# yuecideng/Misc3D

Measured on AMD Instinct MI355X. Metric: RANSAC hypotheses/sec, 1M-pt cloud (inlier-score GB/s: roofline.algorithmic_reuse), higher is better.
Workload: dtype f64 decisions (fp32 screen + fp64 recount)

## Files before the change

### include/misc3d_amd.h

```cpp
#ifndef MISC3D_AMD_H
#define MISC3D_AMD_H

#include <stddef.h>
#include <stdint.h>

#ifdef __cplusplus
extern "C" {
#endif

#define M3D_OK 1
#define M3D_FALSE 0
#define M3D_ERR_PROBABILITY (-1)
#define M3D_ERR_TOO_FEW_POINTS (-2)
#define M3D_ERR_NO_NORMALS (-3)
#define M3D_ERR_SIZE_MISMATCH (-4)
#define M3D_ERR_INVALID_ARG (-5)
#define M3D_ERR_DEVICE (-6)
#define M3D_ERR_INTERNAL (-7)
#define M3D_ERR_NON_FINITE (-8)

enum m3d_model_kind { M3D_PLANE = 0, M3D_SPHERE = 1, M3D_CYLINDER = 2 };

typedef struct m3d_stats {
    double fitness;
// ... 354 lines not shown
    uint64_t n_nodes;
    uint64_t n_rays;
    uint64_t pair_tests;
    uint64_t nodes_visited;
} m3d_raycast_stats;
int m3d_raycast_pinhole(const m3d_raycast_mesh *meshes, size_t n_meshes, const double *poses, size_t n_poses, size_t n_frames,
                        int width, int height, double fx, double fy, double cx, double cy, int device, float *t_hit,
                        uint32_t *geometry_ids, uint32_t *primitive_ids, float *primitive_normals, m3d_raycast_stats *stats);

int m3d_match_mutual_nn(const double *feat_src, size_t n_src, const double *feat_dst, size_t n_dst,
                        int dim, int method, int n_trees, int device, size_t *out_src,
                        size_t *out_dst, size_t *k);
uint64_t m3d_match_last_fallbacks(void);

typedef struct m3d_comm m3d_comm;
#define M3D_COMM_ID_BYTES 128
int m3d_comm_unique_id(uint8_t id[M3D_COMM_ID_BYTES]);
m3d_comm *m3d_comm_create_rccl(const uint8_t id[M3D_COMM_ID_BYTES], int world, int rank, int device);
typedef int (*m3d_allgather_fn)(void *user, const void *send, void *recv, size_t bytes_per_rank);
m3d_comm *m3d_comm_create_host(int world, int rank, m3d_allgather_fn fn, void *user);
int m3d_comm_create_local(int world, m3d_comm **comms );
void m3d_comm_destroy(m3d_comm *comm);
int m3d_comm_world(const m3d_comm *comm);
int m3d_comm_rank(const m3d_comm *comm);
uint64_t m3d_comm_collectives(const m3d_comm *comm);

int m3d_cloud_fit_sharded(m3d_cloud *cloud, m3d_comm *comm, int kind, double threshold, size_t max_iteration,
                          double probability, const uint64_t *seed, double *params, size_t *inliers,
                          size_t *n_inliers, m3d_stats *stats);
int m3d_segment_plane_iterative_sharded(const double *xyz, size_t n, double threshold, int max_iteration,
                                        double min_ratio, const uint64_t *seed, int device, m3d_comm *comm,
                                        size_t max_clusters, double *planes, size_t *cluster_offsets,
                                        size_t *cluster_indices, size_t *n_clusters);
int m3d_segment_plane_iterative_multi(const double *xyz, size_t n, double threshold, int max_iteration,
                                      double min_ratio, const uint64_t *seed, const int *devices, int n_dev,
                                      size_t max_clusters, double *planes, size_t *cluster_offsets,
                                      size_t *cluster_indices, size_t *n_clusters);
int m3d_fit_multi(int kind, const double *xyz, const double *normals, size_t n, double threshold,
                  size_t max_iteration, double probability, const uint64_t *seed, const int *devices, int n_dev,
                  double *params, size_t *inliers, size_t *n_inliers, m3d_stats *stats);
int m3d_registration_ransac_sharded(const double *src, size_t n_src, const double *dst, size_t n_dst,
                                    const size_t *corr_src, const size_t *corr_dst, size_t m, double threshold,
                                    int max_iter, double edge_length_threshold, double confidence,
                                    const uint64_t *seed, int device, m3d_comm *comm, double T[16],
                                    m3d_reg_stats *stats);

typedef struct m3d_config {
    int32_t dense_scoring;
    int32_t speculative_refine;
    int32_t lead_hypotheses;
    int32_t score_groups_per_block;
    int32_t score_min_workgroups;
    int32_t dense_workgroups;
    int32_t reg_neighbour_lists;
    int32_t reg_prune;
    int32_t match_brute;
    int32_t match_fp32_screen;
    int32_t pool_limit_mb;
    int32_t kernel_timing;
    int32_t reg_sorted_lists;
    int32_t score_fp32_screen;
    int32_t cull_fp32;
    int32_t reg_fp32_screen;
    int32_t sorted_tombstones;
    int32_t score_mfma;
    int32_t score_mfma_groups;
    int32_t score_waves4;
    int32_t score_waves4_groups;
    int32_t score_phases;
    int32_t compact_one_pass;
    int32_t plane_bound;
    int32_t lanes;
    int32_t wait_spin_us;
    int32_t prestream;
    int32_t chunk_cap;
    int32_t first_chunk;
    int32_t reg_cells_per_radius;
    int32_t match_pipeline;
    int32_t reg_cache;
    int32_t device_aliases;
    int32_t lanes_eager;
    int32_t list_mask;
    int32_t mask_early;
} m3d_config;
void m3d_get_config(m3d_config *out);
int m3d_set_config(const m3d_config *in);

const char *m3d_last_error(void);
int m3d_device_count(void);
const char *m3d_version(void);

#ifdef __cplusplus
}
#endif
#endif
```

### include/misc3d_amd_bench.h

```cpp
#ifndef MISC3D_AMD_BENCH_H
#define MISC3D_AMD_BENCH_H

#include "misc3d_amd.h"

#ifdef __cplusplus
extern "C" {
#endif

int m3d_bench_time_score(m3d_cloud *cloud, int kind, double threshold, const uint32_t *samples,
                         size_t n_hypotheses, int reps, int mode, double *ms_avg,
                         uint64_t *listed_pairs);


int m3d_bench_fp64_issue_rate(int device, double ms_target, double *tera_lane_ops_per_s, double *ms_measured);

int m3d_bench_cloud_setup_ms(const m3d_cloud *cloud, double out[5]);

int m3d_bench_plane_upper_bounds(m3d_cloud *cloud, double threshold, const uint32_t *samples, size_t n_hypotheses,
                                 uint32_t *ub_out);
int m3d_bench_upper_bounds(m3d_cloud *cloud, int kind, double threshold, const uint32_t *samples, size_t n_hypotheses,
                           uint32_t *ub_out);
int m3d_bench_last_segment_ms(double out[6]);

int m3d_bench_reg_checkers(const double *ps, const double *pd, const double *T, double edge_threshold,
                           double distance_threshold);

int m3d_bench_kabsch_sums(const double *src, const double *dst, size_t n, int device, double out[18]);

int m3d_bench_icp_sums(const double *src, size_t n_src, const double *dst, size_t n_dst, double max_correspondence_distance,
                       const double *T, int device, double out[29], int64_t *corr);

int m3d_bench_fps_force_path(int path);

int m3d_bench_knn_force_path(int path);

int m3d_bench_voxel_force_path(int path);

int m3d_bench_proximity_cutoffs(double dist, double angle_deg, double out[5]);

int m3d_bench_fpfh_pair_bins(const double *pairs, size_t m, int32_t *bins, double *features);

unsigned m3d_bench_match_last_path(void);

#ifdef __cplusplus
}
#endif
#endif
```

### misc3d_amd/capi.py

```python
from __future__ import annotations

import ctypes as C
import threading
import os
import sys
from dataclasses import dataclass

import numpy as np

_HERE = os.path.dirname(os.path.abspath(__file__))
FP_ORDER = int(os.environ.get("M3D_FP_ORDER", "0") or 0)
_VARIANT = os.environ.get("M3D_LIB_VARIANT", "")
LIB_PATH = os.path.join(_HERE, "lib", *([_VARIANT] if _VARIANT else ([f"order{FP_ORDER}"] if FP_ORDER else [])), "libmisc3d_amd.so")
HEADER_PATH = os.path.join(os.path.dirname(_HERE), "include", "misc3d_amd.h")

PLANE, SPHERE, CYLINDER = 0, 1, 2
MINIMAL_SAMPLE = {PLANE: 3, SPHERE: 4, CYLINDER: 2}
NUM_PARAMS = {PLANE: 4, SPHERE: 4, CYLINDER: 7}
MODEL_STRIDE = 8

OK, FALSE = 1, 0
ERR_PROBABILITY, ERR_TOO_FEW_POINTS, ERR_NO_NORMALS, ERR_SIZE_MISMATCH = -1, -2, -3, -4
ERR_INVALID_ARG, ERR_DEVICE, ERR_INTERNAL = -5, -6, -7
ERR_NON_FINITE = -8
# ... 149 lines not shown
                                                  C.c_void_p, C.c_void_p]
        L.m3d_bench_voxel_force_path.argtypes = [C.c_int]
        L.m3d_raycast_pinhole.argtypes = [C.c_void_p, C.c_size_t, C.c_void_p, C.c_size_t, C.c_size_t, C.c_int, C.c_int, C.c_double,
                                          C.c_double, C.c_double, C.c_double, C.c_int, C.c_void_p, C.c_void_p, C.c_void_p,
                                          C.c_void_p, C.c_void_p]
        L.m3d_proximity_segment.argtypes = [C.c_void_p, C.c_void_p, C.c_size_t, C.c_size_t, C.c_double, C.c_void_p,
                                            C.c_size_t, C.c_size_t, C.c_int, C.c_void_p, C.c_void_p, C.c_void_p, C.c_void_p,
                                            C.c_void_p]
        L.m3d_proximity_segment_nn.argtypes = [C.c_void_p, C.c_void_p, C.c_size_t, C.c_size_t, C.c_size_t, C.c_void_p,
                                               C.c_void_p, C.c_void_p, C.c_size_t, C.c_size_t, C.c_int, C.c_void_p,
                                               C.c_void_p, C.c_void_p, C.c_void_p, C.c_void_p]
        L.m3d_radius_neighbors.argtypes = [C.c_void_p, C.c_size_t, C.c_double, C.c_int, C.c_void_p, C.c_void_p, C.c_void_p,
                                           C.c_size_t, C.c_void_p]
        L.m3d_bench_proximity_cutoffs.argtypes = [C.c_double, C.c_double, C.c_void_p]
        L.m3d_knn_create.restype = C.c_void_p
        L.m3d_knn_create.argtypes = [C.c_void_p, C.c_size_t, C.c_int, C.c_int, C.c_void_p]
        L.m3d_knn_destroy.restype = None
        L.m3d_knn_destroy.argtypes = [C.c_void_p]
        L.m3d_knn_size.restype = C.c_size_t
        L.m3d_knn_size.argtypes = [C.c_void_p]
        L.m3d_knn_dim.argtypes = [C.c_void_p]
        L.m3d_knn_search.argtypes = [C.c_void_p, C.c_void_p, C.c_size_t, C.c_int, C.c_int64, C.c_double, C.c_size_t,
                                     C.c_void_p, C.c_void_p, C.c_void_p, C.c_void_p, C.c_void_p]
        L.m3d_bench_knn_force_path.argtypes = [C.c_int]
        L.m3d_estimate_normals.argtypes = [C.c_void_p, C.c_size_t, C.c_int, C.c_double, C.c_int, C.c_int, C.c_void_p, C.c_int,
                                           C.c_void_p, C.c_void_p]
        L.m3d_compute_fpfh.argtypes = [C.c_void_p, C.c_void_p, C.c_size_t, C.c_int, C.c_double, C.c_int, C.c_int, C.c_void_p,
                                       C.c_void_p]
        L.m3d_preprocess_fragment.argtypes = [C.c_void_p, C.c_void_p, C.c_size_t, C.c_double, C.c_int, C.c_void_p, C.c_void_p,
                                              C.c_void_p]
        L.m3d_bench_fpfh_pair_bins.argtypes = [C.c_void_p, C.c_size_t, C.c_void_p, C.c_void_p]
        L.m3d_match_last_fallbacks.restype = C.c_uint64
        L.m3d_match_last_fallbacks.argtypes = []
        L.m3d_match_mutual_nn.argtypes = [C.c_void_p, C.c_size_t, C.c_void_p, C.c_size_t, C.c_int, C.c_int, C.c_int,
                                          C.c_int, C.c_void_p, C.c_void_p, C.c_void_p]
        L.m3d_comm_unique_id.argtypes = [C.c_void_p]
        L.m3d_comm_create_rccl.restype = C.c_void_p
        L.m3d_comm_create_rccl.argtypes = [C.c_void_p, C.c_int, C.c_int, C.c_int]
        L.m3d_comm_create_host.restype = C.c_void_p
        L.m3d_comm_create_host.argtypes = [C.c_int, C.c_int, ALLGATHER_FN, C.c_void_p]
        L.m3d_comm_create_local.argtypes = [C.c_int, C.c_void_p]
        L.m3d_comm_destroy.restype = None
        L.m3d_comm_destroy.argtypes = [C.c_void_p]
        L.m3d_comm_world.argtypes = [C.c_void_p]
        L.m3d_comm_rank.argtypes = [C.c_void_p]
        L.m3d_comm_collectives.restype = C.c_uint64
        L.m3d_comm_collectives.argtypes = [C.c_void_p]
        L.m3d_cloud_fit_sharded.argtypes = [C.c_void_p, C.c_void_p, C.c_int, C.c_double, C.c_size_t, C.c_double, C.c_void_p,
                                            C.c_void_p, C.c_void_p, C.c_void_p, C.c_void_p]
        L.m3d_segment_plane_iterative_clouds.argtypes = [C.c_void_p, C.c_size_t, C.c_double, C.c_int, C.c_double,
                                                          C.c_void_p, C.c_int, C.c_size_t, C.c_void_p, C.c_void_p,
                                                          C.c_void_p, C.c_void_p, C.c_void_p]
        L.m3d_segment_plane_iterative_sharded.argtypes = [C.c_void_p, C.c_size_t, C.c_double, C.c_int, C.c_double,
                                                          C.c_void_p, C.c_int, C.c_void_p, C.c_size_t, C.c_void_p,
                                                          C.c_void_p, C.c_void_p, C.c_void_p]
        L.m3d_segment_plane_iterative_multi.argtypes = [C.c_void_p, C.c_size_t, C.c_double, C.c_int, C.c_double,
                                                        C.c_void_p, C.c_void_p, C.c_int, C.c_size_t, C.c_void_p,
                                                        C.c_void_p, C.c_void_p, C.c_void_p]
        L.m3d_fit_multi.argtypes = [C.c_int, C.c_void_p, C.c_void_p, C.c_size_t, C.c_double, C.c_size_t, C.c_double,
                                    C.c_void_p, C.c_void_p, C.c_int, C.c_void_p, C.c_void_p, C.c_void_p, C.c_void_p]
        L.m3d_registration_ransac_sharded.argtypes = [C.c_void_p, C.c_size_t, C.c_void_p, C.c_size_t, C.c_void_p,
                                                      C.c_void_p, C.c_size_t, C.c_double, C.c_int, C.c_double,
                                                      C.c_double, C.c_void_p, C.c_int, C.c_void_p, C.c_void_p,
                                                      C.c_void_p]
        L.m3d_bench_fp64_issue_rate.argtypes = [C.c_int, C.c_double, C.c_void_p, C.c_void_p]
        L.m3d_bench_cloud_setup_ms.argtypes = [C.c_void_p, C.c_void_p]
        L.m3d_bench_last_segment_ms.argtypes = [C.c_void_p]
        L.m3d_bench_reg_checkers.argtypes = [C.c_void_p, C.c_void_p, C.c_void_p, C.c_double, C.c_double]
        L.m3d_get_config.restype = None
        L.m3d_get_config.argtypes = [C.c_void_p]
        L.m3d_set_config.argtypes = [C.c_void_p]
        L.m3d_release_cached.restype = None
        L.m3d_release_cached.argtypes = [C.c_int]
        _lib = L
    return _lib


class Config(C.Structure):
    _fields_ = [(k, C.c_int32) for k in ("dense_scoring", "speculative_refine", "lead_hypotheses",
                                         "score_groups_per_block", "score_min_workgroups", "dense_workgroups",
                                         "reg_neighbour_lists", "reg_prune", "match_brute", "match_fp32_screen",
                                         "pool_limit_mb", "kernel_timing", "reg_sorted_lists", "score_fp32_screen",
                                         "cull_fp32", "reg_fp32_screen", "sorted_tombstones", "score_mfma", "score_mfma_groups", "score_waves4", "score_waves4_groups", "score_phases", "compact_one_pass", "plane_bound",
                                         "lanes", "wait_spin_us", "prestream", "chunk_cap", "first_chunk", "reg_cells_per_radius", "match_pipeline", "reg_cache", "device_aliases", "lanes_eager", "list_mask", "mask_early")]


def fp64_issue_rate(device=0, ms_target=2.0):
    t, ms = C.c_double(0), C.c_double(0)
    _check(lib().m3d_bench_fp64_issue_rate(device, ms_target, C.cast(C.byref(t), C.c_void_p), C.cast(C.byref(ms), C.c_void_p)))
    return float(t.value), float(ms.value)


def match_last_path() -> int:
    f = lib().m3d_bench_match_last_path
    f.restype = C.c_uint
    f.argtypes = []
    return int(f())


def get_config() -> Config:
    c = Config()
    lib().m3d_get_config(C.byref(c))
    return c


def set_config(**kw) -> Config:
    old = get_config()
    new = get_config()
    for k, v in kw.items():
        if not hasattr(new, k):
            raise AttributeError(k)
        setattr(new, k, int(v))
    _check(lib().m3d_set_config(C.byref(new)))
    return old


def restore_config(cfg: Config):
    _check(lib().m3d_set_config(C.byref(cfg)))


class Comm:

    def __init__(self, handle, keep=None):
        if not handle:
            raise M3DError(ERR_DEVICE, last_error())
        self._h = handle
        self._keep = keep

    @classmethod
    def rccl(cls, group=None, device=0, world=None, rank=None):
        import torch
        import torch.distributed as dist
        if world is None:
            world, rank = (dist.get_world_size(group), dist.get_rank(group)) if dist.is_initialized() else (1, 0)
        ident = np.zeros(128, dtype=np.uint8)
        status = np.zeros(129, dtype=np.uint8)
        err = None
        if rank == 0:
            try:
                _check(lib().m3d_comm_unique_id(_p(ident)))
                status[:128] = ident
                status[128] = 1
            except M3DError as e:
                err = e
        if world > 1:
            t = torch.from_numpy(status)
            dist.broadcast(t, src=dist.get_global_rank(group, 0) if group is not None else 0, group=group)
        if not status[128]:
            raise err if err is not None else M3DError(-6, "rank 0 could not create an RCCL unique id")
        ident = np.ascontiguousarray(status[:128])
        libc = C.CDLL(None)
        sys.stdout.flush()
        libc.fflush(None)
        if os.environ.get("M3D_RCCL_KEEP_STDOUT") == "1":
            return cls(lib().m3d_comm_create_rccl(_p(ident), world, rank, device))
        saved = os.dup(1)
        os.dup2(2, 1)
        try:
            h = lib().m3d_comm_create_rccl(_p(ident), world, rank, device)
        finally:
            libc.fflush(None)
            os.dup2(saved, 1)
            os.close(saved)
        return cls(h)

    @classmethod
    def host(cls, world, rank, fn):
# ... 219 lines not shown
            try:
                self._inl_buf = np.asarray(_PinnedU64(n))
            except MemoryError:
                self._inl_buf = np.empty(n, dtype=np.uint64)
        return self._inl_buf

    def close(self):
        if getattr(self, "_h", None):
            lib().m3d_cloud_destroy(self._h)
            self._h = None
        self._inl_buf = None

    def __del__(self):
        try:
            self.close()
        except Exception:
            pass

    def __enter__(self):
        return self

    def __exit__(self, *a):
        self.close()

    def fit(self, kind, threshold=0.01, max_iteration=1000, probability=0.9999, seed=None,
            want_inliers=True, copy=True) -> Fit:
        params = np.zeros(NUM_PARAMS[kind])
        inl = None
        if want_inliers:
            inl = _seg_scratch(max(self.n_created, 1)) if copy else None
            if inl is None:
                inl = self._out_buf()
        ni = C.c_size_t(0)
        st = Stats()
        _s, sref = _seed_ref(seed)
        rc = _check(lib().m3d_cloud_fit(self._h, kind, threshold, max_iteration, probability, sref, _addr(params),
                                        _addr(inl), C.byref(ni), C.byref(st)))
        if want_inliers:
            inliers = inl[: ni.value].copy() if copy else inl[: ni.value]
        else:
            inliers = np.zeros(0, dtype=np.uint64)
        return Fit(rc, params, inliers, (st, ni.value))

    def fit_sharded(self, comm, kind, threshold=0.01, max_iteration=1000, probability=0.9999, seed=None,
                    want_inliers=True, copy=True) -> Fit:
        params = np.zeros(NUM_PARAMS[kind])
        inl = self._out_buf() if want_inliers else None
        ni = C.c_size_t(0)
        st = Stats()
        _s, sref = _seed_ref(seed)
        rc = _check(lib().m3d_cloud_fit_sharded(self._h, comm._h if comm is not None else None, kind, threshold,
                                                max_iteration, probability, sref, _addr(params), _addr(inl),
                                                C.byref(ni), C.byref(st)))
        if want_inliers:
            inliers = inl[: ni.value].copy() if copy else inl[: ni.value]
        else:
            inliers = np.zeros(0, dtype=np.uint64)
        return Fit(rc, params, inliers, (st, ni.value))

    def score_range(self, kind, threshold, samples, begin=0, end=None, want_models=True):
        samples = np.ascontiguousarray(samples, dtype=np.uint32).reshape(-1, MINIMAL_SAMPLE[kind])
        end = len(samples) if end is None else end
        cnt = np.empty(end - begin, dtype=np.uint32)
        val = np.empty(end - begin, dtype=np.uint8)
        mod = np.empty((end - begin, MODEL_STRIDE)) if want_models else None
        _check(lib().m3d_cloud_score_range(self._h, kind, threshold, _p(samples), begin, end, _p(cnt), _p(val),
                                           _p(mod)))
        return val, (mod[:, : NUM_PARAMS[kind]].copy() if want_models else None), cnt

    def time_score(self, kind, threshold, samples, reps=5, mode=0):
        samples = np.ascontiguousarray(samples, dtype=np.uint32).reshape(-1, MINIMAL_SAMPLE[kind])
        ms = C.c_double(0)
        listed = C.c_uint64(0)
        _check(lib().m3d_bench_time_score(self._h, kind, threshold, _p(samples), len(samples), reps, mode,
                                          C.cast(C.byref(ms), C.c_void_p), C.cast(C.byref(listed), C.c_void_p)))
        return float(ms.value), int(listed.value)

    def plane_upper_bounds(self, threshold, samples):
        samples = np.ascontiguousarray(samples, dtype=np.uint32).reshape(-1, 3)
        ub = np.zeros(len(samples), dtype=np.uint32)
        _check(lib().m3d_bench_plane_upper_bounds(self._h, threshold, _p(samples), len(samples), _p(ub)))
        return ub

    def upper_bounds(self, kind, threshold, samples):
        samples = np.ascontiguousarray(samples, dtype=np.uint32).reshape(-1, MINIMAL_SAMPLE[kind])
        ub = np.zeros(len(samples), dtype=np.uint32)
        _check(lib().m3d_bench_upper_bounds(self._h, kind, threshold, _p(samples), len(samples), _p(ub)))
        return ub

    def exact_error(self, kind, threshold, model):
        model = _f64(model)
        cnt = C.c_uint64(0)
        err = C.c_double(0)
        _check(lib().m3d_cloud_exact_error(self._h, kind, threshold, _p(model), C.cast(C.byref(cnt), C.c_void_p),
                                           C.cast(C.byref(err), C.c_void_p)))
        return int(cnt.value), float(err.value)

    refine_takes_expected = True

    def refine(self, kind, threshold, params, copy=True, expected=None):
        params = _f64(params).copy()
        inl = self._out_buf()
        ni = C.c_size_t(0)
        rc = _check(lib().m3d_cloud_refine_expect(self._h, kind, threshold, _p(params),
                                                  -1 if expected is None else int(expected), _p(inl),
                                                  C.cast(C.byref(ni), C.c_void_p)))
        return rc, params, (inl[: ni.value].copy() if copy else inl[: ni.value])

    def minimal_model(self, kind, threshold, sample_row):
        row = np.ascontiguousarray(sample_row, dtype=np.uint32).reshape(-1)
        if self.n == self.n_created:
            pts = np.ascontiguousarray(self._host_xyz[row])
            nrm = np.ascontiguousarray(self._host_nrm[row]) if self._host_nrm is not None else None
            model = np.zeros(8)
            ok = C.c_uint8(0)
            _check(lib().m3d_minimal_fit(kind, _p(pts), _p(nrm), _p(model), C.cast(C.byref(ok), C.c_void_p)))
            return model[: NUM_PARAMS[kind]].copy()
        _, mod, _ = self.score_range(kind, threshold, row.reshape(1, -1), 0, 1)
        return mod[0]

    def remove_inliers(self, kind, threshold, model):
        model = _f64(model).copy()
        nr = C.c_size_t(0)
        _check(lib().m3d_cloud_remove_inliers(self._h, kind, threshold, _p(model), C.cast(C.byref(nr), C.c_void_p)))
        self.n = int(lib().m3d_cloud_size(self._h))
        return nr.value


def draw_samples(n_points, kind, n_hyp, seed):
    out = np.zeros((n_hyp, MINIMAL_SAMPLE[kind]), dtype=np.uint32)
    _check(lib().m3d_draw_samples(n_points, kind, n_hyp, C.c_uint64(seed), _p(out)))
    return out


def fit(kind, xyz, normals=None, threshold=0.01, max_iteration=1000, probability=0.9999, seed=None,
        device=0, copy=True) -> Fit:
    xyz = _f64(xyz).reshape(-1, 3)
    n = len(xyz)
    params = np.zeros(NUM_PARAMS[kind])
    inl = _seg_scratch(max(n, 1))
    if inl is None:
        inl = np.empty(max(n, 1), dtype=np.uint64)
    ni = C.c_size_t(0)
    st = Stats()
    _s, sref = _seed_ref(seed)
    sp = C.cast(sref, C.c_void_p) if sref else None
    nip, stp = C.cast(C.byref(ni), C.c_void_p), C.cast(C.byref(st), C.c_void_p)
    if kind == CYLINDER:
        nrm = _f64(normals).reshape(-1, 3) if normals is not None else None
        rc = lib().m3d_fit_cylinder(_p(xyz), _p(nrm), n, threshold, max_iteration, probability, sp, device,
                                    _p(params), _p(inl), nip, stp)
    else:
        fn = lib().m3d_fit_plane if kind == PLANE else lib().m3d_fit_sphere
        rc = fn(_p(xyz), n, threshold, max_iteration, probability, sp, device, _p(params), _p(inl), nip, stp)
    _check(rc)
    d = st.asdict()
    d["n_inliers"] = int(ni.value)
    return Fit(rc, params, inl[: ni.value].copy() if copy else inl[: ni.value], d)


_seg_tls = threading.local()
_SEG_SCRATCH_MAX = 1 << 25


def _seg_scratch(n):
    if n > _SEG_SCRATCH_MAX:
# ... 931 lines not shown
```

### misc3d_amd/csrc/m3d_bound.hip

```cpp
#include "m3d_cull_kernels.hpp"

#include <cstdlib>

#include "m3d_bound_fp.hpp"
#include "m3d_config.hpp"
#include "m3d_eig3.hpp"
#include "m3d_fp.hpp"
#include "m3d_wave.hpp"

#pragma clang fp contract(off)

namespace m3d {

constexpr int kFrameLevels = 12;

__global__ __launch_bounds__(64) void tile_frames_k(const double* __restrict__ sx, const double* __restrict__ sy,
                                                     const double* __restrict__ sz, uint32_t n_tiles,
                                                     double* __restrict__ frames, uint16_t* __restrict__ cum) {
    __shared__ float pf[3][kTilePoints];
    __shared__ uint32_t hist[kBoundBins + 2];
    const int lane = threadIdx.x;
    const uint32_t tile = blockIdx.x;
    if (tile >= n_tiles) return;
    constexpr int P = kTilePoints / 64;
// ... 98 lines not shown
        for (int j = 0; j < P; ++j) {
            const double dx = px[j] - c[0], dy = py[j] - c[1], dz = pz[j] - c[2];
            const double w = (dx * e[0] + dy * e[1]) + dz * e[2];
            if (fin[j] && fabs(w) < band) {
                m[0] += 1.0;
                m[1] += dx; m[2] += dy; m[3] += dz;
                m[4] += dx * dx; m[5] += dx * dy; m[6] += dx * dz;
                m[7] += dy * dy; m[8] += dy * dz; m[9] += dz * dz;
            }
        }
#pragma unroll
        for (int k = 0; k < 10; ++k) m[k] = wave_sum(m[k]);
        if (!(m[0] >= 8.0)) break;
        const double in = 1.0 / m[0];
        const double mx = m[1] * in, my = m[2] * in, mz = m[3] * in;
        const double A[9] = {m[4] * in - mx * mx, m[5] * in - mx * my, m[6] * in - mx * mz,
                             m[5] * in - mx * my, m[7] * in - my * my, m[8] * in - my * mz,
                             m[6] * in - mx * mz, m[8] * in - my * mz, m[9] * in - mz * mz};
        double en[3];
        j3x3_smallest_eigvec(A, en);
        if (!((en[0] + en[1] + en[2]) * 0.0 == 0.0)) break;
        e[0] = en[0]; e[1] = en[1]; e[2] = en[2];
        c[0] += mx; c[1] += my; c[2] += mz;
        const double q = (e[0] * (A[0] * e[0] + A[1] * e[1] + A[2] * e[2]) + e[1] * (A[3] * e[0] + A[4] * e[1] + A[5] * e[2])) +
                         e[2] * (A[6] * e[0] + A[7] * e[1] + A[8] * e[2]);
        s = sqrt(fmax(q, 0.0));
        s = fmax(s, 1e-7 * ext);
        band = 3.5 * s;
    }
    const int kmin = (fabs(e[0]) <= fabs(e[1]) && fabs(e[0]) <= fabs(e[2])) ? 0 : (fabs(e[1]) <= fabs(e[2]) ? 1 : 2);
    const double a3[3] = {kmin == 0 ? 1.0 : 0.0, kmin == 1 ? 1.0 : 0.0, kmin == 2 ? 1.0 : 0.0};
    double u[3] = {e[1] * a3[2] - e[2] * a3[1], e[2] * a3[0] - e[0] * a3[2], e[0] * a3[1] - e[1] * a3[0]};
    const double ul = sqrt((u[0] * u[0] + u[1] * u[1]) + u[2] * u[2]);
    u[0] /= ul; u[1] /= ul; u[2] /= ul;
    const double v[3] = {e[1] * u[2] - e[2] * u[1], e[2] * u[0] - e[0] * u[2], e[0] * u[1] - e[1] * u[0]};
    const double wlo = -5.0 * s, invd = (double)kBoundBins / (10.0 * s);
    double U = 0.0, V = 0.0, W = 0.0, R = 0.0;
#pragma unroll
    for (int j = 0; j < P; ++j) {
        if (!fin[j]) continue;
        const double dx = px[j] - c[0], dy = py[j] - c[1], dz = pz[j] - c[2];
        const double w = (dx * e[0] + dy * e[1]) + dz * e[2];
        const double uu = (dx * u[0] + dy * u[1]) + dz * u[2];
        const double vv = (dx * v[0] + dy * v[1]) + dz * v[2];
        const double rx = ((dx - w * e[0]) - uu * u[0]) - vv * v[0];
        const double ry = ((dy - w * e[1]) - uu * u[1]) - vv * v[1];
        const double rz = ((dz - w * e[2]) - uu * u[2]) - vv * v[2];
        U = fmax(U, fabs(uu));
        V = fmax(V, fabs(vv));
        W = fmax(W, fabs(w));
        R = fmax(R, fmax(fabs(rx), fmax(fabs(ry), fabs(rz))));
        atomicAdd(&hist[bound_bin(w, wlo, invd)], 1u);
    }
    U = wave_max(U);
    V = wave_max(V);
    W = wave_max(W);
    R = wave_max(R);
    __syncthreads();
    {
        const uint32_t h0 = hist[2 * lane], h1 = hist[2 * lane + 1];
        const uint32_t own = h0 + h1, incl = wave_incl_scan(own, lane);
        const uint32_t excl = incl - own;
        cm[2 * lane] = (uint16_t)excl;
        cm[2 * lane + 1] = (uint16_t)(excl + h0);
        if (lane == 63) cm[kBoundBins + 2] = (uint16_t)incl;
    }
    const double Rm = R + 1e-13 * (mabs + ext);
    const bool ok = (U + V + W + Rm) < 1e12 && invd > 0.0 && invd < 1e30 && ext > 1e-12 && mabs < 1e12;
    if (lane == 0) {
        fr[0] = c[0]; fr[1] = c[1]; fr[2] = c[2];
        fr[3] = e[0]; fr[4] = e[1]; fr[5] = e[2];
        fr[6] = u[0]; fr[7] = u[1]; fr[8] = u[2];
        fr[9] = v[0]; fr[10] = v[1]; fr[11] = v[2];
        fr[12] = U; fr[13] = V; fr[14] = Rm; fr[15] = wlo; fr[16] = invd; fr[17] = W; fr[18] = nf;
        fr[19] = ok ? 1.0 : 0.0;
    }
}

void launch_tile_frames(const SortedView& s, double* frames, uint16_t* cum, hipStream_t st) {
    if (s.n_tiles) tile_frames_k<<<s.n_tiles, 64, 0, st>>>(s.x, s.y, s.z, s.n_tiles, frames, cum);
}

constexpr int kBoundWaves = 8;
template <int KIND , int kBoundTpw >
__global__ __launch_bounds__(64 * kBoundWaves) void plane_bound_k(const double* __restrict__ frames, const uint16_t* __restrict__ cum,
                                                                   uint32_t n_tiles, double max_abs,
                                                                   const double* __restrict__ score,
                                                                   const unsigned long long* __restrict__ masks, uint32_t n_groups,
                                                                   const double* __restrict__ boxes, const float* __restrict__ cull32,
                                                                   uint32_t* __restrict__ surv_count,
                                                                   const uint32_t* __restrict__ surv,
                                                                   uint32_t* __restrict__ ubsum, const uint32_t* __restrict__ best_count,
                                                                   unsigned long long* __restrict__ keep,
                                                                   uint32_t* __restrict__ tickets ,
                                                                   uint32_t max_list) {
    constexpr int kBoundTpb = kBoundWaves * kBoundTpw;
    __shared__ float bx_s[kBoundTpb][6];
    __shared__ double c_s[kBoundTpb][3];
    __shared__ float f_s[kBoundTpb][kFrameStride];
    __shared__ __attribute__((aligned(8))) uint16_t cm_s[kBoundTpb][kCumStride];
    __shared__ uint32_t wsum[kBoundWaves][64];
    __shared__ double rec_s[64][9];
    __shared__ float q_s[64][13];
    const int lane = threadIdx.x & 63;
    const int wave = __builtin_amdgcn_readfirstlane((int)(threadIdx.x >> 6));
    const uint32_t total = surv_count[0];
    if (total > max_list) {
        if (blockIdx.x == 0 && blockIdx.y == 0 && threadIdx.x == 0) surv_count[0] = 0u;
        return;
    }
    if (blockIdx.x * 64u >= total) return;
    const uint32_t t0 = blockIdx.y * (uint32_t)kBoundTpb, nt = min((uint32_t)kBoundTpb, n_tiles - t0);
    {
        const double* __restrict__ src = frames + (size_t)t0 * kFrameStride;
        for (uint32_t i = threadIdx.x; i < nt * (uint32_t)kFrameStride; i += 64u * kBoundWaves) {
            const uint32_t tl = i / (uint32_t)kFrameStride, k = i % (uint32_t)kFrameStride;
            const double v = src[i];
            if (k < 3u) c_s[tl][k] = v;
            f_s[tl][k] = frame_to_f32(v, k);
        }
        if (KIND != 0) {
            __syncthreads();
            if (threadIdx.x < nt) f_s[threadIdx.x][0] = cyl_tile_rho(f_s[threadIdx.x]);
        }
        if (cull32)
            for (uint32_t i = threadIdx.x; i < nt * 6u; i += 64u * kBoundWaves)
                bx_s[i / 6u][i % 6u] = reinterpret_cast<const float*>(boxes + (size_t)(t0 + i / 6u) * kBoxStride + 8)[i % 6u];
        const uint32_t* __restrict__ csrc = reinterpret_cast<const uint32_t*>(cum + (size_t)t0 * kCumStride);
        uint32_t* cdst = reinterpret_cast<uint32_t*>(&cm_s[0][0]);
        for (uint32_t i = threadIdx.x; i < nt * (uint32_t)(kCumStride / 2); i += 64u * kBoundWaves) cdst[i] = csrc[i];
    }
    for (uint32_t first = blockIdx.x * 64u; first < total; first += gridDim.x * 64u) {
        const uint32_t nb = min(64u, total - first);
        const bool has = (uint32_t)lane < nb;
        const uint32_t h = surv[first + (has ? (uint32_t)lane : 0u)];
        __syncthreads();
        {
            const uint32_t k = threadIdx.x & 7u;
#pragma unroll
            for (uint32_t si = threadIdx.x >> 3; si < 64u; si += (64u * kBoundWaves) >> 3) {
                const uint32_t hh = surv[first + min(si, nb - 1u)];
                rec_s[si][k] = score[(size_t)hh * kModelStride + k];
                if (cull32) {
                    q_s[si][k] = cull32[(size_t)(hh >> 1) * 24u + (hh & 1u) + 2u * k];
                    if (KIND == 2 && k < 3u) q_s[si][8u + k] = cull32[(size_t)(hh >> 1) * 24u + (hh & 1u) + 2u * (8u + k)];
                }
            }
        }
        __syncthreads();
        PlaneBoundRec pr;
        CylBoundRec cr;
        if (KIND == 0) {
            pr = plane_bound_record(rec_s[lane], max_abs);
            pr.ok = pr.ok && has;
        } else {
            cr = KIND == 1 ? sphere_bound_record(rec_s[lane], max_abs) : cyl_bound_record(rec_s[lane], max_abs);
            cr.ok = cr.ok && has;
        }
        const unsigned long long bit = 1ull << (h & 63u);
        const unsigned long long* __restrict__ mrow = masks + (size_t)(h >> 6);
        bool tch[kBoundTpw];
        float q[11] = {0, 0, 0, 0, 0, 0, 0, 0, 0, 0, 0};
        if (cull32) {
#pragma unroll
            for (int k = 0; k < (KIND == 2 ? 11 : 8); ++k) q[k] = q_s[lane][k];
        } else {
#pragma unroll
            for (int i = 0; i < kBoundTpw; ++i) {
                const uint32_t tl = (uint32_t)(wave + kBoundWaves * i);
                tch[i] = (has && tl < nt) ? (mrow[(size_t)(t0 + tl) * n_groups] & bit) != 0ull : false;
            }
        }
        uint32_t ub = 0;
#pragma unroll
        for (int i = 0; i < kBoundTpw; ++i) {
            const int tl = wave + kBoundWaves * i;
            if (cull32 && KIND == 0) {
                const float* bx = bx_s[tl];
                const float sv = __builtin_fmaf(q[0], bx[0], __builtin_fmaf(q[1], bx[1], __builtin_fmaf(q[2], bx[2], q[3])));
                const float hx = __builtin_fmaxf(bx[3], 0.0f), hy = __builtin_fmaxf(bx[4], 0.0f), hz = __builtin_fmaxf(bx[5], 0.0f);
                const float rv = __builtin_fmaf(q[4], hx, __builtin_fmaf(q[5], hy, __builtin_fmaf(q[6], hz, q[7])));
                tch[i] = has && (uint32_t)tl < nt && bx[3] >= 0.0f && !(rv - __builtin_fabsf(sv) < 0.0f);
            } else if (cull32 && KIND == 2) {
                const float* bx = bx_s[tl];
                const bool live = bx[3] >= 0.0f;
                const float hx = live ? bx[3] : 0.0f, hy = live ? bx[4] : 0.0f, hz = live ? bx[5] : 0.0f;
                const float rb = __builtin_sqrtf(__builtin_fmaf(hz, hz, __builtin_fmaf(hy, hy, hx * hx))) * 1.000001f;
                const float d1 = __builtin_fmaf(q[0], bx[0], __builtin_fmaf(q[1], bx[1], __builtin_fmaf(q[2], bx[2], q[3])));
                const float d2 = __builtin_fmaf(q[4], bx[0], __builtin_fmaf(q[5], bx[1], __builtin_fmaf(q[6], bx[2], q[7])));
                const float tt = __builtin_fmaf(d2, d2, d1 * d1);
                const float dist = __builtin_sqrtf(tt);
                const float rt = q[8] * rb;
                const float t1 = (q[9] + rt) - dist;
                const float t2 = (dist + rt) - q[10];
                const float t = __uint_as_float(__float_as_uint(t1) | __float_as_uint(t2));
                tch[i] = has && (uint32_t)tl < nt && live && !(t < 0.0f);
            }
            if (__ballot(tch[i]) == 0ull) continue;
            const uint32_t u_t = KIND == 0 ? plane_pair_ub(pr, c_s[tl], f_s[tl], cm_s[tl])
                                           : cyl_pair_ub(cr, c_s[tl], f_s[tl], f_s[tl][0], cm_s[tl]);
            ub += tch[i] ? u_t : 0u;
        }
        wsum[wave][lane] = ub;
        __syncthreads();
        if (wave == 0) {
            uint32_t tot = 0;
#pragma unroll
            for (int w = 0; w < kBoundWaves; ++w) tot += wsum[w][lane];
            if (has && tot) atomicAdd(&ubsum[h], tot);
            __threadfence();
            const uint32_t blk = first / 64u;
            uint32_t old = 0;
            if (lane == 0) old = atomicAdd(&tickets[1u + blk], 1u);
            old = (uint32_t)__builtin_amdgcn_readfirstlane((int)old);
            if (old == gridDim.y - 1u) {
                __threadfence();
                const uint32_t best = best_count[0];
                const uint32_t sum = has ? atomicAdd(&ubsum[h], 0u) : 0u;
                if (has && best != 0u && sum < best) atomicAnd(&keep[h >> 6], ~bit);
                uint32_t done = 0;
                if (lane == 0) {
                    tickets[1u + blk] = 0u;
                    done = atomicAdd(&tickets[0], 1u);
                    if (done == (total + 63u) / 64u - 1u) {
                        tickets[0] = 0u;
                        surv_count[0] = 0u;
                    }
                }
            }
        }
    }
}

constexpr int kCylTpb = 64;
__global__ __launch_bounds__(64 * kBoundWaves) void cyl_bound_words_k(const double* __restrict__ frames, const uint16_t* __restrict__ cum,
                                                                       uint32_t n_tiles, double max_abs, const double* __restrict__ score,
                                                                       uint32_t* __restrict__ surv_count, const uint32_t* __restrict__ surv,
                                                                       uint32_t* __restrict__ ubsum, const uint32_t* __restrict__ best_count,
                                                                       unsigned long long* __restrict__ keep, uint32_t* __restrict__ tickets,
                                                                       uint32_t max_list, const unsigned long long* __restrict__ touched,
                                                                       uint32_t touched_stride) {
    __shared__ double c_s[kCylTpb][3];
    __shared__ float f_s[kCylTpb][kFrameStride];
    __shared__ __attribute__((aligned(8))) uint16_t cm_s[kCylTpb][kCumStride];
    const int lane = threadIdx.x & 63;
    const uint32_t wave = threadIdx.x >> 6;
    const uint32_t total = surv_count[0];
    if (total > max_list) {
        if (blockIdx.x == 0 && blockIdx.y == 0 && threadIdx.x == 0) surv_count[0] = 0u;
        return;
    }
    if (blockIdx.x * (64u * kBoundWaves) >= total) return;
    const uint32_t t0 = blockIdx.y * (uint32_t)kCylTpb, nt = min((uint32_t)kCylTpb, n_tiles - t0);
    {
        const double* __restrict__ src = frames + (size_t)t0 * kFrameStride;
        for (uint32_t i = threadIdx.x; i < nt * (uint32_t)kFrameStride; i += 64u * kBoundWaves) {
            const uint32_t tl = i / (uint32_t)kFrameStride, k = i % (uint32_t)kFrameStride;
            const double v = src[i];
            if (k < 3u) c_s[tl][k] = v;
            f_s[tl][k] = frame_to_f32(v, k);
        }
        __syncthreads();
        if (threadIdx.x < nt) f_s[threadIdx.x][0] = cyl_tile_rho(f_s[threadIdx.x]);
        const uint32_t* __restrict__ csrc = reinterpret_cast<const uint32_t*>(cum + (size_t)t0 * kCumStride);
        uint32_t* cdst = reinterpret_cast<uint32_t*>(&cm_s[0][0]);
        for (uint32_t i = threadIdx.x; i < nt * (uint32_t)(kCumStride / 2); i += 64u * kBoundWaves) cdst[i] = csrc[i];
        __syncthreads();
    }
    for (uint32_t first = (blockIdx.x * kBoundWaves + wave) * 64u; first < total; first += gridDim.x * (64u * kBoundWaves)) {
        const uint32_t nb = min(64u, total - first);
        const bool has = (uint32_t)lane < nb;
        const uint32_t h = surv[first + (has ? (uint32_t)lane : 0u)];
        double rec[8];
        {
            const double2* __restrict__ rp = reinterpret_cast<const double2*>(score + (size_t)h * kModelStride);
#pragma unroll
            for (int k = 0; k < 4; ++k) {
                const double2 v = rp[k];
                rec[2 * k] = v.x;
                rec[2 * k + 1] = v.y;
            }
        }
        CylBoundRec cr = cyl_bound_record(rec, max_abs);
        cr.ok = cr.ok && has;
        unsigned long long w0 = has ? touched[(size_t)(t0 / 64u) * touched_stride + h] : 0ull;
        unsigned long long w1 = (has && t0 + 64u < n_tiles) ? touched[(size_t)(t0 / 64u + 1u) * touched_stride + h] : 0ull;
        uint32_t ub = 0;
        for (uint32_t tl = 0; tl < nt; ++tl) {
            const bool mine = (((tl < 64u ? w0 : w1) >> (tl & 63u)) & 1ull) != 0ull;
            if (__builtin_amdgcn_ballot_w64(mine) == 0ull) continue;
            const uint32_t u_t = cyl_pair_ub(cr, c_s[tl], f_s[tl], f_s[tl][0], cm_s[tl]);
            ub += mine ? u_t : 0u;
        }
        if (has && ub) atomicAdd(&ubsum[h], ub);
        __threadfence();
        const uint32_t blk = first / 64u;
        uint32_t old = 0;
        if (lane == 0) old = atomicAdd(&tickets[1u + blk], 1u);
        old = (uint32_t)__builtin_amdgcn_readfirstlane((int)old);
        if (old == gridDim.y - 1u) {
            __threadfence();
            const uint32_t best = best_count[0];
            const uint32_t sum = has ? atomicAdd(&ubsum[h], 0u) : 0u;
            if (has && best != 0u && sum < best) atomicAnd(&keep[h >> 6], ~(1ull << (h & 63u)));
            if (lane == 0) {
                tickets[1u + blk] = 0u;
                const uint32_t done = atomicAdd(&tickets[0], 1u);
                if (done == (total + 63u) / 64u - 1u) {
                    tickets[0] = 0u;
                    surv_count[0] = 0u;
                }
            }
        }
    }
}

void launch_plane_bound(int kind, const SortedView& s, const double* score, const unsigned long long* masks, unsigned long long* keep,
                        uint32_t n_groups, uint32_t group_begin, uint32_t group_end, uint32_t* ubsum,
                        const uint32_t* best_count, uint32_t* surv_count, const uint32_t* surv, uint32_t* tickets,
                        const float* cull32, hipStream_t st, bool always, const unsigned long long* touched, uint32_t touched_stride) {
    group_end = std::min(group_end, n_groups);
    if (!s.frames || !s.frame_cum || !s.n_tiles || !surv || !surv_count || !tickets || group_begin >= group_end) return;
    const uint32_t window = group_end - group_begin;
    constexpr uint32_t gdiv = 6;
    const uint32_t gx = std::min<uint32_t>(window, std::max<uint32_t>(4u, (window + gdiv - 1) / gdiv));
    constexpr int tpw = 8, tpw_cyl = 16;
    const uint32_t tpb = (uint32_t)(kBoundWaves * (kind == 0 ? tpw : tpw_cyl));
    const uint32_t max_list = always ? 0xFFFFFFFFu : window * 32u;
    if (kind == 2 && touched && s.radius < 1e18) {
        const dim3 gw((window + kBoundWaves - 1) / kBoundWaves, (s.n_tiles + kCylTpb - 1) / kCylTpb);
        cyl_bound_words_k<<<gw, 64 * kBoundWaves, 0, st>>>(s.frames, s.frame_cum, s.n_tiles, s.max_abs, score, surv_count, surv, ubsum, best_count,
                                                           keep, tickets, max_list, touched, touched_stride);
        return;
    }
    const dim3 g(gx, (s.n_tiles + tpb - 1) / tpb), b(64 * kBoundWaves);
    if (s.radius >= 1e18 || kind == 1) cull32 = nullptr;
    auto go = [&](auto kernel) {
        kernel<<<g, b, 0, st>>>(s.frames, s.frame_cum, s.n_tiles, s.max_abs, score, masks, n_groups, s.boxes, cull32, surv_count, surv,
                                ubsum, best_count, keep, tickets, max_list);
    };
    if (kind == 0) go(plane_bound_k<0, tpw>);
    else if (kind == 1) go(plane_bound_k<1, tpw_cyl>);
    else go(plane_bound_k<2, tpw_cyl>);
}

}
```

### misc3d_amd/csrc/m3d_bound_fp.hpp

```cpp
#pragma once
#include <math.h>
#include <stdint.h>

#if defined(__HIPCC__)
#include <hip/hip_runtime.h>
#ifndef M3D_HD
#define M3D_HD __host__ __device__ __forceinline__
#endif
#else
#ifndef M3D_HD
#define M3D_HD inline
#endif
#endif

namespace m3d {

constexpr int kFrameStride = 20;
constexpr int kBoundBins = 126;
constexpr int kCumStride = 132;
constexpr int kBoundTilePoints = 512;

M3D_HD int bound_bin(double w, double wlo, double invd) {
    const double t = floor((w - wlo) * invd);
    return (int)fmin(fmax(t, -1.0), (double)kBoundBins) + 1;
// ... 95 lines not shown
    return r;
}
M3D_HD CylBoundRec sphere_bound_record(const double* rec , double max_abs) {
    CylBoundRec r;
    const double Wm = 2.0 * max_abs + ((fabs(rec[0]) + fabs(rec[1])) + fabs(rec[2]));
    const double Es = 1e-12 * (Wm * Wm);
    const double slo = rec[3], shi = rec[4];
    r.ok = (slo == slo) && (shi == shi) && (shi >= 0.0) && (Wm < 1e12) && (shi < 1e30);
    for (int k = 0; k < 3; ++k) {
        r.p1[k] = rec[k];
        r.df[k] = 0.0f;
    }
    const double dhi = sqrt(shi + Es) * (1.0 + 1e-12);
    const double sl = slo - Es;
    const double dlo = sl > 0.0 ? sqrt(sl) * (1.0 - 1e-12) : 0.0;
    r.dhif = (float)(dhi * (1.0 + 1e-6));
    r.dlof = (float)(dlo * (1.0 - 1e-6));
    r.mg = (float)(1e-13 * Wm * (1.0 + 1e-6));
    return r;
}
M3D_HD float bound_sqrt(float x) {
#if defined(__HIP_DEVICE_COMPILE__)
    return __builtin_amdgcn_sqrtf(x);
#else
    return sqrtf(x);
#endif
}
M3D_HD float cyl_tile_rho(const float* f) {
    const float U = f[12], V = f[13], R = f[14], W = f[17];
    return __builtin_fmaf(bound_sqrt(__builtin_fmaf(W, W, __builtin_fmaf(U, U, V * V))), 1.0001f, 1.75f * R);
}
template <class CumPtr>
M3D_HD uint32_t cyl_pair_ub(const CylBoundRec& r, const double* c3, const float* f, float rho, CumPtr cm) {
    const float U = f[12], V = f[13], R = f[14], W = f[17];
    const bool framed = f[19] != 0.0f && r.ok;
    const float v0 = (float)(c3[0] - r.p1[0]), v1 = (float)(c3[1] - r.p1[1]), v2 = (float)(c3[2] - r.p1[2]);
    const float v1n = (__builtin_fabsf(v0) + __builtin_fabsf(v1)) + __builtin_fabsf(v2);
    const float k = __builtin_fmaf(v0, r.df[0], __builtin_fmaf(v1, r.df[1], v2 * r.df[2]));
    const float m0 = __builtin_fmaf(-k, r.df[0], v0), m1 = __builtin_fmaf(-k, r.df[1], v1), m2 = __builtin_fmaf(-k, r.df[2], v2);
    const float f2 = __builtin_fmaf(m0, m0, __builtin_fmaf(m1, m1, m2 * m2));
    const float fc = bound_sqrt(f2);
    const float eabs = 2e-6f * v1n;
    const bool one_side = fc - eabs > rho * 1.001f && f2 < 1e30f && f2 > 1e-30f;
    const float inv = bound_rcp(fc);
    const float nx = m0 * inv, ny = m1 * inv, nz = m2 * inv;
    const float n1 = 1.7321f, e32 = 5e-7f * 1.7321f;
    const float g0 = __builtin_fmaf(nx, f[3], __builtin_fmaf(ny, f[4], nz * f[5]));
    const float nu = __builtin_fmaf(nx, f[6], __builtin_fmaf(ny, f[7], nz * f[8]));
    const float nv = __builtin_fmaf(nx, f[9], __builtin_fmaf(ny, f[10], nz * f[11]));
    const float hif = r.dhif - fc;
    const float rho1 = rho * 1.0001f;
    const float q2 = __builtin_fmaf(r.dlof, r.dlof, -(rho1 * rho1)) - 3e-7f * (r.dlof * r.dlof);
    const bool has_lo = q2 > 1e-30f;
    const float lof = has_lo ? bound_sqrt(q2) * (1.0f - 3e-7f) - fc : 0.0f;
    float aa = __builtin_fmaf(__builtin_fabsf(nu) + e32, U,
                              __builtin_fmaf(__builtin_fabsf(nv) + e32, V, __builtin_fmaf(n1, R, __builtin_fmaf(e32, W, r.mg + eabs))));
    aa = __builtin_fmaf(aa, 1.00001f, 1e-5f * ((__builtin_fabsf(hif) + __builtin_fabsf(lof)) + aa));
#ifdef M3D_BOUND_NO_SLACK
    aa = 0.0f;
#endif
    const float ninf = -__builtin_huge_valf();
    const float g = __builtin_fabsf(g0);
    const float a_lo = g0 < 0.0f ? -hif : (has_lo ? lof : ninf), a_hi = g0 < 0.0f ? (has_lo ? -lof : -ninf) : hif;
    const float ig = bound_rcp(g);
    float Lw = (a_lo - aa) * ig, Hw = (a_hi + aa) * ig;
    Lw -= 1e-5f * __builtin_fabsf(Lw);
    Hw += 1e-5f * __builtin_fabsf(Hw);
    const float wlo = f[15], invd = f[16];
#ifdef M3D_BOUND_NO_SLACK
    const float out = 0.0f;
#else
    const float out = 1.0f;
#endif
    const float tL = __builtin_floorf((Lw - wlo) * invd) - out, tH = __builtin_floorf((Hw - wlo) * invd) + out;
    const bool whole = !(tL == tL) || !(tH == tH) || !one_side;
    const int bl = (int)__builtin_fminf(__builtin_fmaxf(whole ? 0.0f : tL, -1.0f), (float)kBoundBins) + 1;
    const int bh = (int)__builtin_fminf(__builtin_fmaxf(whole ? 0.0f : tH, -1.0f), (float)kBoundBins) + 1;
    const int lo_c = (int)cm[bl], hi_c = (int)cm[bh + 1];
    uint32_t u_t = (uint32_t)(hi_c > lo_c ? hi_c - lo_c : 0);
    u_t = whole ? (uint32_t)f[18] : u_t;
    return framed ? u_t : (uint32_t)kBoundTilePoints;
}

}
```

### misc3d_amd/csrc/m3d_config.cpp

```cpp
#include "m3d_config.hpp"

#include <algorithm>
#include <cstdlib>
#include <cstring>
#include <mutex>

#include "m3d_driver.hpp"

namespace m3d {
namespace {
m3d_config g_cfg;
std::once_flag g_once;
std::mutex g_cfg_mu;
thread_local m3d_config t_cfg;
thread_local int t_cfg_pins = 0;

long env_long(const char* name, long def) {
    const char* e = std::getenv(name);
    if (!e || !*e) return def;
    char* end = nullptr;
    const long v = std::strtol(e, &end, 10);
    return end == e ? def : v;
}
bool env_is(const char* name, char first) {
    const char* e = std::getenv(name);
    return e && e[0] == first;
}
void sanitize(m3d_config& c) {
    if (c.lead_hypotheses < 64 || c.lead_hypotheses % 64) c.lead_hypotheses = 128;
    if (c.score_groups_per_block < 1 || c.score_groups_per_block > 64) c.score_groups_per_block = 8;
    if (c.score_min_workgroups < 1) c.score_min_workgroups = 8192;
    if (c.dense_workgroups < 1) c.dense_workgroups = 8192;
    if (c.pool_limit_mb < 0) c.pool_limit_mb = 0;
    if (c.score_phases < -1 || c.score_phases == 1 || c.score_phases > 3) c.score_phases = -1;
    if (c.plane_bound < 0 || c.plane_bound > 2) c.plane_bound = 1;
    if (c.cull_fp32 < 0 || c.cull_fp32 > 2) c.cull_fp32 = 1;
    c.score_mfma = c.score_mfma_groups = c.score_waves4 = c.score_waves4_groups = c.compact_one_pass = 0;
    if (c.lanes < 1 || c.lanes > 8) c.lanes = 4;
    if (c.wait_spin_us < 0) c.wait_spin_us = 500;
    c.prestream = c.prestream != 0;
    c.chunk_cap = (int32_t)std::min<long>(std::max<long>(((long)c.chunk_cap + 63) / 64 * 64, 1024), 262144);
    c.first_chunk = c.first_chunk <= 0 ? 0 : (int32_t)std::min<long>(((long)c.first_chunk + 63) / 64 * 64, 1 << 20);
    if (c.reg_cells_per_radius < 1 || c.reg_cells_per_radius > 16) c.reg_cells_per_radius = 4;
    if (c.match_pipeline < 0 || c.match_pipeline > 2) c.match_pipeline = 1;
    if (c.reg_cache < 0 || c.reg_cache > 2) c.reg_cache = 1;
    if (c.device_aliases < 0) c.device_aliases = 0;
    if (c.device_aliases > 16) c.device_aliases = 16;
    if (c.lanes_eager < 1 || c.lanes_eager > 8) c.lanes_eager = 2;
    if (c.list_mask < 0) c.list_mask = 1;
    if (c.list_mask > 16) c.list_mask = 16;
    c.mask_early = c.mask_early != 0;
}
void load_env() {
    std::memset(&g_cfg, 0, sizeof(g_cfg));
    g_cfg.dense_scoring = env_is("M3D_DENSE", '1');
    g_cfg.speculative_refine = !env_is("M3D_SPEC", '0');
    g_cfg.lead_hypotheses = (int32_t)env_long("M3D_LEAD", 128);
    g_cfg.score_groups_per_block = (int32_t)env_long("M3D_GPB", 8);
    g_cfg.score_min_workgroups = (int32_t)env_long("M3D_SCORE_MIN_WGS", 8192);
    g_cfg.dense_workgroups = (int32_t)env_long("M3D_SCORE_WGS", 8192);
    g_cfg.reg_neighbour_lists = !env_is("M3D_REG_NL", '0');
    g_cfg.reg_prune = !env_is("M3D_REG_PRUNE", '0');
    g_cfg.match_brute = env_is("M3D_MATCH_BRUTE", '1');
    g_cfg.match_fp32_screen = env_is("M3D_MATCH_SCREEN", 'f');
    g_cfg.pool_limit_mb = (int32_t)env_long("M3D_POOL_MB", 4096);
    g_cfg.kernel_timing = env_is("M3D_KERNEL_TIMING", '1');
    g_cfg.reg_sorted_lists = !env_is("M3D_REG_SORTED", '0');
    g_cfg.score_fp32_screen = !env_is("M3D_SCORE_SCREEN", '0');
    g_cfg.cull_fp32 = env_is("M3D_CULL_FP32", '0') ? 0 : (env_is("M3D_CULL_FP32", '2') ? 2 : 1);
    g_cfg.reg_fp32_screen = !env_is("M3D_REG_SCREEN", '0');
    g_cfg.sorted_tombstones = !env_is("M3D_TOMBSTONES", '0');
    g_cfg.score_phases = (int32_t)env_long("M3D_SCORE_PHASES", -1);
    g_cfg.plane_bound = (int32_t)env_long("M3D_PLANE_BOUND", 1);
    g_cfg.lanes = (int32_t)env_long("M3D_LANES", 4);
    g_cfg.wait_spin_us = (int32_t)env_long("M3D_SPIN_US", 500);
    g_cfg.prestream = !env_is("M3D_PRESTREAM", '0');
    g_cfg.chunk_cap = (int32_t)env_long("M3D_CHUNK_CAP", 24576);
    g_cfg.first_chunk = (int32_t)env_long("M3D_FIRST_CHUNK", 2048);
    g_cfg.reg_cells_per_radius = (int32_t)env_long("M3D_REG_K", 4);
    g_cfg.match_pipeline = (int32_t)env_long("M3D_MATCH_PIPELINE", 1);
    g_cfg.reg_cache = (int32_t)env_long("M3D_REG_CACHE", 1);
    g_cfg.device_aliases = (int32_t)env_long("M3D_DEVICE_ALIASES", 0);
    g_cfg.lanes_eager = (int32_t)env_long("M3D_LANES_EAGER", 2);
    g_cfg.list_mask = (int32_t)env_long("M3D_LIST_MASK", 1);
    g_cfg.mask_early = !env_is("M3D_MASK_EARLY", '0');
    sanitize(g_cfg);
}
}

const m3d_config& config() {
    std::call_once(g_once, load_env);
    if (t_cfg_pins > 0) return t_cfg;
    std::lock_guard<std::mutex> lock(g_cfg_mu);
    t_cfg = g_cfg;
    return t_cfg;
}
void config_pin() {
    std::call_once(g_once, load_env);
    if (t_cfg_pins++ == 0) {
        std::lock_guard<std::mutex> lock(g_cfg_mu);
        t_cfg = g_cfg;
    }
}
void config_unpin() {
    if (t_cfg_pins > 0) --t_cfg_pins;
}
void config_store(const m3d_config& c) {
    std::call_once(g_once, load_env);
    m3d_config n = c;
    sanitize(n);
    std::lock_guard<std::mutex> lock(g_cfg_mu);
    g_cfg = n;
}
}

extern "C" {
void m3d_get_config(m3d_config* out) {
    if (out) *out = m3d::config();
}
int m3d_set_config(const m3d_config* in) {
    if (!in) return m3d::fail(M3D_ERR_INVALID_ARG, "invalid argument");
    if (in->score_mfma || in->score_waves4 || in->compact_one_pass)
        return m3d::fail(M3D_ERR_INVALID_ARG, "score_mfma / score_waves4 / compact_one_pass: retired, must be 0 (the variants were removed)");
    m3d::config_store(*in);
    return M3D_OK;
}
}
```

### misc3d_amd/csrc/m3d_cull_kernels.hip

```cpp
#include "m3d_cull_kernels.hpp"
#include "m3d_poison.hpp"

#include <hip/hip_ext.h>

#include <cstdlib>
#include <type_traits>

#include "m3d_config.hpp"
#include "m3d_fp.hpp"
#include "m3d_tile_count.hpp"
#include "m3d_wave.hpp"

#pragma clang fp contract(off)

namespace m3d {

typedef float f32x2 __attribute__((ext_vector_type(2)));

__global__ __launch_bounds__(256) void tile_boxes_k(const double* __restrict__ sx, const double* __restrict__ sy,
                                                     const double* __restrict__ sz, uint32_t n_tiles,
                                                     double* __restrict__ boxes, double ox, double oy, double oz,
                                                     float* __restrict__ tile_f32) {
    const int lane = threadIdx.x & 63;
    const uint32_t tile = blockIdx.x * 4u + (threadIdx.x >> 6);
    if (tile >= n_tiles) return;
    double lo[3] = {INFINITY, INFINITY, INFINITY}, hi[3] = {-INFINITY, -INFINITY, -INFINITY};
    double pts[kTilePoints / 64][3];
#pragma unroll
    for (int j = 0; j < kTilePoints / 64; ++j) {
        const size_t i = (size_t)tile * kTilePoints + j * 64 + lane;
        const double p[3] = {sx[i], sy[i], sz[i]};
        for (int k = 0; k < 3; ++k) {
            pts[j][k] = p[k];
            lo[k] = fmin(lo[k], p[k]);
            hi[k] = fmax(hi[k], p[k]);
        }
    }
    for (int off = 32; off > 0; off >>= 1)
        for (int k = 0; k < 3; ++k) {
            lo[k] = fmin(lo[k], __shfl_xor(lo[k], off, 64));
            hi[k] = fmax(hi[k], __shfl_xor(hi[k], off, 64));
        }
    bool finite = true;
    if (tile_f32) {
        const bool empty_t = !(lo[0] <= hi[0]);
        f32x2* __restrict__ t2 = reinterpret_cast<f32x2*>(tile_f32 + (size_t)tile * kTileF32Floats);
#pragma unroll
        for (int k = 0; k < 3; ++k) {
            const double c = empty_t ? 0.0 : 0.5 * lo[k] + 0.5 * hi[k];
#pragma unroll
            for (int j = 0; j < kTilePoints / 128; ++j) {
                const f32x2 v = {(float)(pts[2 * j][k] - c), (float)(pts[2 * j + 1][k] - c)};
                t2[(k * (kTilePoints / 128) + j) * 64 + lane] = v;
                finite = finite && (v.x * 0.0f == 0.0f) && (v.y * 0.0f == 0.0f);
            }
        }
    }
    const bool screenable = tile_f32 && __ballot(!finite) == 0ull;
    if (lane == 0) {
        double* b = boxes + (size_t)tile * kBoxStride;
        const bool empty = !(lo[0] <= hi[0]);
        for (int k = 0; k < 3; ++k) {
            const double c = 0.5 * lo[k] + 0.5 * hi[k];
            b[k] = empty ? 0.0 : c;
            b[3 + k] = empty ? -1.0 : fmax(hi[k] - c, c - lo[k]) * (1.0 + 1e-12) + 1e-300;
        }
        b[6] = screenable ? 1.0 : 0.0;
        b[7] = 0.0;
        float* f = reinterpret_cast<float*>(b + 8);
        const double o[3] = {ox, oy, oz};
        for (int k = 0; k < 3; ++k) {
            const double cr = b[k] - o[k];
            const float c32 = (float)cr;
            const double hh = (b[3 + k] + fabs(cr - (double)c32)) * (1.0 + 1e-6) + 1e-30;
            f[k] = empty ? 0.0f : c32;
            f[3 + k] = empty ? -1.0f : f32_round_up(hh);
        }
        const float hx = empty ? 0.0f : f[3], hy = empty ? 0.0f : f[4], hz = empty ? 0.0f : f[5];
        f[6] = __builtin_sqrtf(__builtin_fmaf(hz, hz, __builtin_fmaf(hy, hy, hx * hx))) * 1.000001f;
        f[7] = 0.0f;
    }
}

void launch_tile_boxes(const SortedView& s, double* boxes, hipStream_t st) {
    if (s.n_tiles) tile_boxes_k<<<(s.n_tiles + 3) / 4, 256, 0, st>>>(s.x, s.y, s.z, s.n_tiles, boxes, s.origin[0], s.origin[1], s.origin[2], s.tile_f32);
}

__global__ __launch_bounds__(256) void poison_plane_inliers_k(PoisonJob job) {
    poison_tile(job, blockIdx.x * 4u + (threadIdx.x >> 6), (int)(threadIdx.x & 63));
}
PoisonJob make_poison_job(const SortedView& s, const double* model, double thr, uint32_t* total) {
    PoisonJob j;
// ... 338 lines not shown
    if (!s.n_tiles || group_begin >= group_end) return;
    const uint32_t window = group_end - group_begin;
    if (ub && !ub_is_zero) (void)hipMemsetAsync(ub + (size_t)group_begin * 64, 0, sizeof(uint32_t) * (size_t)window * 64, st);
    const uint32_t tblocks = (s.n_tiles + 63) / 64;
    uint32_t gpw = std::max<uint32_t>(1, (uint32_t)(((uint64_t)tblocks * window) / 8192));
    gpw = std::min<uint32_t>(gpw, 8);
    const dim3 g(tblocks, (window + gpw - 1) / gpw), b(64);
    if (cull32 && s.radius < 1e18 && config().cull_fp32 != 0) {
        if (window >= 128u && config().cull_fp32 != 2) {
            const uint32_t tpw = 64u;
            const dim3 gh((s.n_tiles + tpw - 1) / tpw, window);
            if (kind == 0) cull_hyp32_k<0><<<gh, b, 0, st>>>(s.boxes, s.n_tiles, cull32, n_groups, tpw, masks, ub, group_begin, group_end, ubp, touched, touched_stride);
            else if (kind == 1) cull_hyp32_k<1><<<gh, b, 0, st>>>(s.boxes, s.n_tiles, cull32, n_groups, tpw, masks, ub, group_begin, group_end, ubp, touched, touched_stride);
            else cull_hyp32_k<2><<<gh, b, 0, st>>>(s.boxes, s.n_tiles, cull32, n_groups, tpw, masks, ub, group_begin, group_end, ubp, touched, touched_stride);
            if (touched_written) *touched_written = touched != nullptr;
            return;
        }
        if (kind == 0)
            cull_tiles32_k<0><<<g, b, 0, st>>>(s.boxes, s.n_tiles, cull32, n_groups, gpw, masks, ub, group_begin, group_end, ubp);
        else if (kind == 1)
            cull_tiles32_k<1><<<g, b, 0, st>>>(s.boxes, s.n_tiles, cull32, n_groups, gpw, masks, ub, group_begin, group_end, ubp);
        else
            cull_tiles32_k<2><<<g, b, 0, st>>>(s.boxes, s.n_tiles, cull32, n_groups, gpw, masks, ub, group_begin, group_end, ubp);
        return;
    }
    if (kind == 0)
        cull_tiles_k<0><<<g, b, 0, st>>>(s.boxes, s.n_tiles, score, n_groups, gpw, masks, ub, group_begin, group_end);
    else if (kind == 1)
        cull_tiles_k<1><<<g, b, 0, st>>>(s.boxes, s.n_tiles, score, n_groups, gpw, masks, ub, group_begin, group_end);
    else
        cull_tiles_k<2><<<g, b, 0, st>>>(s.boxes, s.n_tiles, score, n_groups, gpw, masks, ub, group_begin, group_end);
}

struct SurvOut {
    uint32_t* count = nullptr;
    uint32_t* ids = nullptr;
};
__device__ __forceinline__ void emit_survivors(const SurvOut surv, unsigned long long m, bool k, uint32_t h) {
    if (!surv.count || !m) return;
    uint32_t base = 0;
    if (threadIdx.x == 0) base = atomicAdd(surv.count, (uint32_t)__popcll(m));
    base = (uint32_t)__builtin_amdgcn_readfirstlane((int)base);
    const uint32_t rank = __builtin_amdgcn_mbcnt_hi((uint32_t)(m >> 32), __builtin_amdgcn_mbcnt_lo((uint32_t)m, 0u));
    if (k) surv.ids[base + rank] = h;
}
__global__ __launch_bounds__(64) void keep_mask_k(const uint32_t* __restrict__ ub,
                                                   const uint32_t* __restrict__ best_count_ptr,
                                                   unsigned long long* __restrict__ keep,
                                                   uint32_t* __restrict__ zero, uint32_t rep_stride,
                                                   uint32_t group_offset, SurvOut surv) {
    const uint32_t g = group_offset + blockIdx.x;
    const uint32_t h = g * 64u + threadIdx.x;
    const uint32_t best = best_count_ptr ? best_count_ptr[0] : 0u;
    const bool k = !ub || best == 0 || (uint64_t)ub[h] * kTilePoints >= best;
    const unsigned long long m = __ballot(k);
    if (threadIdx.x == 0) keep[g] = m;
    emit_survivors(surv, m, k, h);
    if (zero) {
#pragma unroll
        for (int r = 0; r < kCountReplicas; ++r) zero[(size_t)r * rep_stride + h] = 0u;
        if (blockIdx.x == 0)
            for (int i = threadIdx.x; i < kPairReplicas; i += 64) zero[(size_t)kCountReplicas * rep_stride + i] = 0u;
    }
}
void launch_keep_mask(const uint32_t* ub, const uint32_t* best_count, uint32_t n_groups, unsigned long long* keep,
                      hipStream_t st, uint32_t* zero_counts_rep, uint32_t rep_stride, uint32_t group_offset, uint32_t* surv_count, uint32_t* surv) {
    if (!n_groups) return;
    if (!ub && !zero_counts_rep && !surv_count) {
        (void)hipMemsetAsync(keep + group_offset, 0xFF, sizeof(unsigned long long) * n_groups, st);
        return;
    }
    keep_mask_k<<<n_groups, 64, 0, st>>>(ub, best_count, keep, zero_counts_rep, rep_stride, group_offset, SurvOut{surv_count, surv});
}

__global__ __launch_bounds__(64) void lead_fold_keep_k(const uint32_t* __restrict__ counts_rep, uint32_t rep_stride,
                                                        uint32_t lead, const uint8_t* __restrict__ valid, uint32_t h_count,
                                                        uint32_t* __restrict__ records, uint32_t* __restrict__ best_count,
                                                        const uint32_t* __restrict__ ub,
                                                        unsigned long long* __restrict__ keep,
                                                        uint32_t* __restrict__ zero, uint32_t group_offset,
                                                        uint32_t* __restrict__ records_dev,
                                                        unsigned long long* __restrict__ pick_key,
                                                        unsigned long long* __restrict__ pick_key2,
                                                        SurvOut surv) {
    const uint32_t g = group_offset + blockIdx.x;
    const uint32_t prev = best_count[0];
    uint32_t v = 0;
    unsigned long long key = 0, key2 = 0;
    for (uint32_t h = threadIdx.x; h < lead; h += 64u) {
        uint32_t c = 0;
#pragma unroll
        for (int r = 0; r < kCountReplicas; ++r) c += counts_rep[(size_t)r * rep_stride + h];
        const bool ok = h < h_count && valid[h];
        if (blockIdx.x == 0) {
            if (records) records[h] = c | (ok ? 0x80000000u : 0u);
            if (records_dev) records_dev[h] = c | (ok ? 0x80000000u : 0u);
        }
        v = max(v, ok ? c : 0u);
        if (ok && c) key = max(key, ((unsigned long long)c << 32) | (0xFFFFFFFFu - h));
        if (ok && c) key2 = max(key2, ((unsigned long long)c << 32) | h);
    }
    v = wave_max(v);
    if (blockIdx.x == 0 && threadIdx.x == 0 && v) atomicMax(best_count, v);
    if (zero && blockIdx.x == 0) {
        uint32_t* __restrict__ pair_rep = zero + (size_t)kCountReplicas * rep_stride;
        uint32_t p = 0;
        for (int r = threadIdx.x; r < kPairMain; r += 64) p += pair_rep[r];
        p = wave_sum(p);
        if (threadIdx.x == 0) pair_rep[kPairLead] = p;
    }
    if (pick_key && blockIdx.x == 0) {
        key = wave_max(key);
        if (threadIdx.x == 0 && key) atomicMax(pick_key, key);
        if (pick_key2) {
            key2 = wave_max(key2);
            if (threadIdx.x == 0 && key2) atomicMax(pick_key2, key2);
        }
    }
    const uint32_t best = max(prev, v);
    const uint32_t h = g * 64u + threadIdx.x;
    const bool k = !ub || best == 0 || (uint64_t)ub[h] * kTilePoints >= best;
    const unsigned long long m = __ballot(k);
    if (threadIdx.x == 0) keep[g] = m;
    emit_survivors(surv, m, k, h);
    if (zero) {
#pragma unroll
        for (int r = 0; r < kCountReplicas; ++r) zero[(size_t)r * rep_stride + h] = 0u;
    }
}
void launch_lead_fold_keep(const uint32_t* counts_rep, uint32_t rep_stride, uint32_t lead, const uint8_t* valid,
                           uint32_t h_count, uint32_t* records, uint32_t* best_count, const uint32_t* ub,
                           unsigned long long* keep, uint32_t n_groups_rest, hipStream_t st, uint32_t* records_dev,
                           uint32_t group_begin, unsigned long long* pick_key, unsigned long long* pick_key2, uint32_t* surv_count, uint32_t* surv) {
    if (group_begin == 0xFFFFFFFFu) group_begin = lead / 64u;
    if (!n_groups_rest) return;
    lead_fold_keep_k<<<n_groups_rest, 64, 0, st>>>(counts_rep, rep_stride, lead, valid, h_count, records, best_count, ub,
                                                   keep, const_cast<uint32_t*>(counts_rep), group_begin, records_dev, pick_key, pick_key2, SurvOut{surv_count, surv});
}

template <int KIND>
__global__ __launch_bounds__(64) void score_mask_k(const double* __restrict__ sx, const double* __restrict__ sy,
                                                    const double* __restrict__ sz,
                                                    const double* __restrict__ score,
                                                    const unsigned long long* __restrict__ masks,
                                                    const unsigned long long* __restrict__ keep,
                                                    uint32_t n_groups ,
                                                    uint32_t groups_per_block,
                                                    uint32_t* __restrict__ counts_rep, uint32_t rep_stride,
                                                    uint32_t* __restrict__ pair_rep,
                                                    uint32_t group_begin, uint32_t group_end ) {
    __shared__ uint16_t ids[64 * 64];
    const uint32_t tile = blockIdx.x;
    uint32_t* __restrict__ counts = counts_rep + (size_t)(tile % kCountReplicas) * rep_stride;
    const uint32_t g0 = group_begin + blockIdx.y * groups_per_block;
    const int lane = threadIdx.x;
    unsigned long long mm = 0;
    if ((uint32_t)lane < groups_per_block && g0 + lane < group_end)
        mm = masks[(size_t)tile * n_groups + g0 + lane] & keep[g0 + lane];
    if (!__ballot(mm != 0)) return;
    const size_t base = (size_t)tile * kTilePoints + lane;
    constexpr int P = kTilePoints / 64;
    double x[P], y[P], z[P];
#pragma unroll
    for (int j = 0; j < P; ++j) {
        x[j] = sx[base + 64 * j];
        y[j] = sy[base + 64 * j];
        z[j] = sz[base + 64 * j];
    }
    const int mm_lo = (int)(uint32_t)mm, mm_hi = (int)(uint32_t)(mm >> 32);
    uint32_t total = 0;
    for (uint32_t w = 0; w < groups_per_block; ++w) {
        const uint32_t lo = (uint32_t)__builtin_amdgcn_readlane(mm_lo, (int)w), hi = (uint32_t)__builtin_amdgcn_readlane(mm_hi, (int)w);
        if ((lo | hi) == 0u) continue;
        const unsigned long long word = ((unsigned long long)hi << 32) | lo;
        const uint32_t below = __builtin_amdgcn_mbcnt_hi(hi, __builtin_amdgcn_mbcnt_lo(lo, 0u));
        if ((word >> lane) & 1ull) ids[total + below] = (uint16_t)(w * 64u + (uint32_t)lane);
        total += (uint32_t)__popcll(word);
    }
    __syncthreads();
    if (lane == 0) atomicAdd(&pair_rep[(tile + blockIdx.y * 67u) % (uint32_t)kPairMain], total);
    constexpr int kUsed = KIND == 2 ? 8 : 5;
    const double* __restrict__ score0 = score + (size_t)g0 * 64u * kModelStride;
    auto load_rec = [&](double (&r)[kModelStride], uint32_t id) {
        const double* __restrict__ rp = score0 + (size_t)id * kModelStride;
#pragma unroll
        for (int k = 0; k < kUsed; ++k) r[k] = rp[k];
    };
    for (uint32_t b0 = 0; b0 < total; b0 += 64u) {
        const uint32_t nb = min(64u, total - b0);
        const int my = (b0 + (uint32_t)lane < total) ? (int)ids[b0 + lane] : 0;
        uint32_t park = 0;
        double ra[kModelStride], rb[kModelStride];
        load_rec(ra, (uint32_t)__builtin_amdgcn_readlane(my, 0));
        for (uint32_t k = 0; k < nb; k += 2u) {
            load_rec(rb, (uint32_t)__builtin_amdgcn_readlane(my, (int)min(k + 1u, nb - 1u)));
            const uint32_t ca = tile_count<KIND, P>(ra, x, y, z);
            park = ((uint32_t)lane == k) ? ca : park;
            load_rec(ra, (uint32_t)__builtin_amdgcn_readlane(my, (int)min(k + 2u, nb - 1u)));
            if (k + 1u < nb) {
                const uint32_t cb = tile_count<KIND, P>(rb, x, y, z);
                park = ((uint32_t)lane == k + 1u) ? cb : park;
            }
        }
        if ((uint32_t)lane < nb && park) atomicAdd(&counts[g0 * 64u + (uint32_t)my], park);
    }
}

#ifndef M3D_SCREEN_MAX_GROUPS
#define M3D_SCREEN_MAX_GROUPS 16
#endif
constexpr uint32_t kScreenMaxGroups = M3D_SCREEN_MAX_GROUPS;
static uint32_t screen_gpb_max(uint32_t window, bool thinned = false) {
    const uint32_t g = (uint32_t)config().score_groups_per_block;
    return std::min<uint32_t>(window >= 192u ? 2u * g : (thinned ? g + g / 2u : g), kScreenMaxGroups);
}
constexpr int kCntStride = 64;

template <int KIND, int Q>
__device__ __forceinline__ void screen_eval(const float4 ra, const float4 rb, const float4 rc, const f32x2 (&xf)[Q],
                                            const f32x2 (&yf)[Q], const f32x2 (&zf)[Q], const f32x2 (&wf)[Q] ,
// ... 660 lines not shown
```

### misc3d_amd/csrc/m3d_cull_kernels.hpp

```cpp
#pragma once
#include "m3d_bound_fp.hpp"
#include "m3d_kernels.hpp"

namespace m3d {

constexpr int kTilePoints = 512;
constexpr int kBoxStride = 12;
constexpr int kCull32Stride = 12;
constexpr uint32_t kGroupsPerBlock = 8;

struct SortedView {
    const double* x;
    const double* y;
    const double* z;
    const double* boxes;
    uint32_t n_tiles;
    float* tile_f32 = nullptr;
    const double* frames = nullptr;
    const uint16_t* frame_cum = nullptr;
    bool has_dead = false;
    double max_abs = __builtin_inf();
    double origin[3] = {0.0, 0.0, 0.0};
    double radius = __builtin_inf();
};

constexpr int kTileF32Floats = 3 * kTilePoints;
void launch_tile_frames(const SortedView& s, double* frames, uint16_t* cum, hipStream_t st);
void launch_plane_bound(int kind, const SortedView& s, const double* score, const unsigned long long* masks, unsigned long long* keep,
                        uint32_t n_groups, uint32_t group_begin, uint32_t group_end, uint32_t* ubsum,
                        const uint32_t* best_count, uint32_t* surv_count, const uint32_t* surv, uint32_t* tickets,
                        const float* cull32, hipStream_t st,
                        bool always = false ,
                        const unsigned long long* touched = nullptr ,
                        uint32_t touched_stride = 0);
void launch_tile_boxes(const SortedView& s, double* boxes, hipStream_t st);
PoisonJob make_poison_job(const SortedView& s, const double* model, double thr, uint32_t* total);
void launch_poison_plane_inliers(const PoisonJob& job, hipStream_t st);


void launch_cull_mask(int kind, const SortedView& s, const double* score, const uint8_t* valid, uint32_t h_count,
                      uint32_t n_groups, unsigned long long* masks, uint32_t* ub, hipStream_t st,
                      bool ub_is_zero = false, uint32_t group_begin = 0,
                      uint32_t group_end = 0xFFFFFFFFu ,
                      const float* cull32 = nullptr ,
                      uint32_t* ubp = nullptr ,
                      unsigned long long* touched = nullptr ,
                      uint32_t touched_stride = 0, bool* touched_written = nullptr );
void launch_keep_mask(const uint32_t* ub, const uint32_t* best_count, uint32_t n_groups, unsigned long long* keep,
                      hipStream_t st, uint32_t* zero_counts_rep = nullptr, uint32_t rep_stride = 0,
                      uint32_t group_offset = 0 ,
                      uint32_t* surv_count = nullptr, uint32_t* surv = nullptr );
constexpr int kCountReplicas = 16;
constexpr int kPairReplicas = 1024;
constexpr int kPairLead = kPairReplicas - 1;
constexpr int kPairMain = 1008;
void launch_score_mask(int kind, const SortedView& s, const double* score, const unsigned long long* masks,
                       const unsigned long long* keep, uint32_t n_groups, uint32_t* counts_rep, uint32_t rep_stride,
                       uint32_t* pair_rep ,
                       hipStream_t st, uint32_t group_begin = 0, uint32_t group_end = 0xFFFFFFFFu ,
                       hipEvent_t ev_start = nullptr, hipEvent_t ev_stop = nullptr ,
                       bool thinned = false );
bool launch_cull_lead(int kind, const SortedView& s, const double* score, const float* cull32, unsigned long long* masks,
                      const unsigned long long* keep, uint32_t n_groups, uint32_t lead_groups, uint32_t* counts_rep,
                      uint32_t rep_stride, uint32_t* pair_rep, uint32_t* ub, uint32_t cull_end, hipStream_t st, uint32_t* ubp = nullptr);
int score_phases_for(int kind);
bool launch_score_phased(int kind, const SortedView& s, const double* score, const unsigned long long* masks,
                         unsigned long long* keep, uint32_t n_groups, uint32_t* counts_rep, uint32_t rep_stride,
                         uint32_t* pair_rep, const uint32_t* ub, const uint32_t* ubp, const uint32_t* best_count, hipStream_t st,
                         uint32_t group_begin, uint32_t group_end, hipEvent_t ev_start, hipEvent_t ev_stop);
struct BestPick {
    unsigned long long index;
    uint32_t cnt, have;
    double params[8];
    uint32_t tie, pad;
};
struct BestPickHost {
    unsigned long long index;
    uint32_t cnt, have;
    uint32_t seq, tie;
};
struct PickFinal {
    unsigned long long* key = nullptr;
    unsigned long long* key2 = nullptr;
    uint32_t* ticket = nullptr;
    const double* params = nullptr;
    unsigned long long index_base = 0;
    int first_chunk = 0;
    BestPick* pick = nullptr;
    BestPickHost* pick_host = nullptr;
    uint32_t seq = 0;
};
void launch_sum_replicas(const uint32_t* counts_rep, uint32_t rep_stride, uint32_t h_end, uint32_t* counts,
                         const uint32_t* pair_rep, uint32_t* pairs_out, const uint8_t* valid, uint32_t h_count,
                         uint32_t* best_count, hipStream_t st, uint32_t h_begin = 0 ,
                         uint32_t* counts_dev = nullptr ,
                         const PickFinal* pick = nullptr,
                         const unsigned long long* keep_final = nullptr );
void launch_pick_best(const uint32_t* records, uint32_t count, unsigned long long index_base, const double* params,
                      bool first_chunk, BestPick* pick, BestPickHost* pick_host, hipStream_t st,
                      uint32_t* records_host = nullptr ,
                      uint32_t* best_count = nullptr );
void launch_lead_fold_keep(const uint32_t* counts_rep, uint32_t rep_stride, uint32_t lead, const uint8_t* valid,
                           uint32_t h_count, uint32_t* records, uint32_t* best_count, const uint32_t* ub,
                           unsigned long long* keep, uint32_t n_groups_rest, hipStream_t st,
                           uint32_t* records_dev = nullptr,
                           uint32_t group_begin = 0xFFFFFFFFu ,
                           unsigned long long* pick_key = nullptr ,
                           unsigned long long* pick_key2 = nullptr ,
                           uint32_t* surv_count = nullptr, uint32_t* surv = nullptr );
void launch_count_bits(const unsigned long long* masks, const unsigned long long* keep, uint32_t n_tiles,
                       uint32_t n_groups, unsigned long long* total, hipStream_t st);

}
```

### misc3d_amd/csrc/m3d_driver.hpp

```cpp
#pragma once
#include <hip/hip_runtime.h>

#include <cstddef>
#include <cstdint>
#include <functional>
#include <mutex>
#include <string>
#include <vector>

#include "../../include/misc3d_amd.h"
#include "m3d_cull_kernels.hpp"
#include "m3d_grid_geom.hpp"
#include "m3d_kernels.hpp"
#include "m3d_reg_kernels.hpp"

struct m3d_cloud;

namespace m3d {

void set_error(const std::string& msg);
int fail(int code, const std::string& msg);

struct DevBuf {
    void* p = nullptr;
// ... 42 lines not shown
    launch_grid_scatter(v, cs.cell.as<uint32_t>(), cs.start.as<uint32_t>(), cs.rank.as<uint32_t>(), qx, qy, qz, s);
}

struct ChunkSlot {
    DevBuf samples, score, params, valid, counts;
    DevBuf cull32;
    DevBuf touched;
    DevBuf masks, ub;
    hipEvent_t pre_done = nullptr;
    PinBuf h_samples, h_counts, h_valid;
    bool lead_fused = false;
    hipEvent_t done = nullptr;
    hipEvent_t k0 = nullptr, k1 = nullptr;
    hipEvent_t k2 = nullptr, k3 = nullptr;
    uint32_t lead_groups = 0;
    bool host_has_records = true;
    bool done_on_copy_stream = false;
    bool scored = false;
    uint32_t poll_seq = 0;
    size_t begin = 0, end = 0;
    uint32_t h_pad = 0;
};

struct DeviceCtx {
    int device = -1;
    int logical = -1;
    int lane = 0;
    hipStream_t stream = nullptr;
    hipStream_t copy_stream = nullptr;
    hipStream_t pre_stream = nullptr;
    hipEvent_t ev_compact = nullptr;
    std::mutex mu;
    ChunkSlot slot[2];
    DevBuf partial, block_counts, total, idx, dist, sum_partial, sums, best_params, small;
    DevBuf masks, keep;
    DevBuf ub, best_count;
    DevBuf counts_rep;
    PinBuf h_small;
    PinBuf h_tie;
    DevBuf tie_scratch;
    void* seg_staging = nullptr;
    size_t seg_staging_cap = 0;
    PinBuf h_inc;
    uint32_t pick_seq = 0;
    const double* last_best_dev = nullptr;
    DevBuf cc_stage, cc_bbox;
    CellSort cc_sort;
    DevBuf pick;
    PinBuf h_pick;
    bool spec_compaction = false;
    uint64_t* idx_out_override = nullptr;
    bool defer_copy_sync = false;
    bool no_prune_hint = false;
    bool defer_refine = false;
    int refine_slot = 0;
    struct DeferredRefine {
        bool pending = false;
        int slot = 0;
        uint32_t ni = 0;
        double* params_out = nullptr;
    } deferred;
    PoisonJob pending_poison;
    bool poison_pending = false;
    uint64_t* poison_expected_at = nullptr, poison_pending_count = 0;
    DevBuf poison_total;
    bool ev_compact_early = false;
    bool spec_hit = false;
    PinBuf h_sums;
    DevBuf moment_partial;
    PinBuf h_moments;
    hipEvent_t ev_pre_gate = nullptr;
    bool compaction_fused = false;
    uint64_t* compaction_idx_host = nullptr;
    bool compaction_mask = false;
    PinBuf h_mask, h_tile_counts;
    uint32_t mask_seq = 0;
    bool compaction_mask_early = false;
    const std::function<const m3d::PartitionOut*(int64_t)>* partition_hook = nullptr;
    PinBuf h_best;
    PinBuf h_sync;
    PinBuf h_reg;
    uint32_t sync_seq = 0;
    DevBuf surv_list;
    hipEvent_t ev0 = nullptr, ev1 = nullptr;
    PinBuf h_match;
    std::vector<hipEvent_t> aux_events;
};

constexpr int kMaxLanes = 8;
struct MatchSide {
    const double* host;
    const double* dev;
    double max_abs;
};
int match_mutual_nn_on(DeviceCtx* ctx, const MatchSide& feat_src, size_t n_src, const MatchSide& feat_dst, size_t n_dst, int dim,
                       size_t* out_src, size_t* out_dst, size_t* k_out);
int device_max_abs(DeviceCtx* ctx, const double* dev, size_t n, double* out);
int registration_ransac_on(DeviceCtx* ctx, m3d_cloud* csrc, m3d_cloud* cdst, const double* src, size_t n_src,
                           const double* dst, size_t n_dst, const size_t* corr_src, const size_t* corr_dst, size_t m,
                           double threshold, int max_iter, double edge_length_threshold, double confidence,
                           const uint64_t* seed, double* T_out, m3d_reg_stats* stats,
                           m3d_reg** session_out = nullptr );
int information_matrix_on(DeviceCtx* ctx, m3d_cloud* csrc, m3d_cloud* cdst, const double* dst, size_t n_dst,
                          double max_correspondence_distance, const double* T, double* info, uint64_t* n_correspondences,
                          m3d_reg* session = nullptr);
void reg_session_release(m3d_reg* q);
inline constexpr char kIcpInvalidDistance[] = "Invalid max_correspondence_distance.";
inline constexpr char kIcpNeedsNormals[] =
    "TransformationEstimationPointToPlane and TransformationEstimationColoredICP require pre-computed normal vectors for target "
    "PointCloud.";
inline constexpr char kIcpNeedsColors[] = "TransformationEstimationForColoredICP requires colors for the source and the target PointCloud.";
inline constexpr char kIcpBadLambda[] = "lambda_geometric must be in [0, 1].";
int registration_icp_on(DeviceCtx* held, const double* src, size_t n_src, const double* dst, size_t n_dst,
                        double max_correspondence_distance, const double* T_init, int max_iteration, double relative_fitness,
                        double relative_rmse, int device, double* T_out, m3d_icp_stats* stats, int64_t* correspondences);
int registration_icp_plane_on(DeviceCtx* held, const double* src, size_t n_src, const double* dst, const double* dst_normals,
                              size_t n_dst, double max_correspondence_distance, const double* T_init, int max_iteration,
                              double relative_fitness, double relative_rmse, int device, double* T_out, m3d_icp_stats* stats,
                              int64_t* correspondences);
int registration_icp_colored_on(DeviceCtx* held, const double* src, const double* src_colors, size_t n_src, const double* dst,
                                const double* dst_normals, const double* dst_colors, size_t n_dst,
                                double max_correspondence_distance, double lambda_geometric, const double* T_init,
                                int max_iteration, double relative_fitness, double relative_rmse, int device, double* T_out,
                                m3d_icp_stats* stats, int64_t* correspondences);
int voxel_levels_on(DeviceCtx* ctx, const double* xyz, const double* normals, size_t n, const double* voxel_sizes, size_t n_levels,
                    double* const* out_xyz, double* const* out_normals, size_t* m, double* level_ms,
                    const double* colors = nullptr, double* const* out_colors = nullptr );
int voxel_sizes_check(const double* voxel_sizes, size_t n_levels);

void dev_pool_trim(int device);
int logical_device_count();
int physical_device(int logical);
DeviceCtx* get_ctx(int device);
DeviceCtx* get_lane(int device, int lane);
hipStream_t copy_stream_of(DeviceCtx* ctx);
hipStream_t pre_stream_of(DeviceCtx* ctx);
hipEvent_t aux_event_of(DeviceCtx* ctx, size_t k);
int lanes_held();
int lane_count();

class CtxLock {
public:
    explicit CtxLock(DeviceCtx* c);
    ~CtxLock();
    CtxLock(const CtxLock&) = delete;
    CtxLock& operator=(const CtxLock&) = delete;

private:
    DeviceCtx* ctx_;
    int prev_lane_, prev_dev_;
};
class LaneLock {
public:
    explicit LaneLock(int device, int prefer = -1);
    ~LaneLock();
    LaneLock(const LaneLock&) = delete;
    LaneLock& operator=(const LaneLock&) = delete;
    DeviceCtx* ctx = nullptr;

private:
    int prev_lane_ = 0, prev_dev_ = -1;
};

}

struct m3d_cloud {
// ... 48 lines not shown
```

### misc3d_amd/csrc/m3d_fit.cpp

```cpp
#include "m3d_driver_internal.hpp"
#include "m3d_generalfit_fp.hpp"

#pragma clang fp contract(off)

namespace m3d {

static uint64_t double_to_size_t_x86(double v) {
    const double two63 = 9223372036854775808.0;
    if (v >= two63) {
        const double w = v - two63;
        if (!(w < two63)) return 0;
        return static_cast<uint64_t>(static_cast<int64_t>(w)) ^ 0x8000000000000000ull;
    }
    if (!(v > -two63)) return 0x8000000000000000ull;
    return static_cast<uint64_t>(static_cast<int64_t>(v));
}

template <class TieFn, class BestFn>
static void replay_range(m3d_replay_state* st, size_t n_points, int kind, size_t max_iteration,
                         double probability, size_t begin, size_t end, const uint8_t* valid,
                         const uint32_t* counts, TieFn tie, BestFn on_best) {
    const bool packed = valid == nullptr;
    const int m = minimal_sample(kind);
    for (size_t i = begin; i < end; ++i) {
// ... 40 lines not shown
                                    size_t begin, size_t end, const uint32_t* rec, TieFn tie, BestFn on_best) {
    if (st->stopped || end <= begin) return;
    const size_t n = end - begin;
    uint32_t mx = 0, nvalid = 0;
    for (size_t k = 0; k < n; ++k) {
        const uint32_t r = rec[k], v = r >> 31, c = r & 0x7FFFFFFFu;
        nvalid += v;
        const uint32_t cv = v ? c : 0u;
        mx = cv > mx ? cv : mx;
    }
    if (mx >= n_points || st->count > st->current_iteration || st->count + nvalid > st->current_iteration) {
        replay_range(st, n_points, kind, max_iteration, 1.0, begin, end, nullptr, rec, tie, on_best);
        return;
    }
    if (mx > 0 && mx >= st->best_count) {
        const uint32_t want = mx | 0x80000000u;
        for (size_t k = 0; k < n; ++k) {
            if (rec[k] != want) continue;
            const size_t i = begin + k;
            const double fitness = (double)mx / (double)n_points;
            bool better = fitness > st->best_fitness;
            double trial_rmse = 0.0;
            bool trial_rmse_known = false;
            if (!better && fitness == st->best_fitness) better = tie(i, mx, &trial_rmse, &trial_rmse_known);
            if (better) {
                st->best_fitness = fitness;
                st->best_rmse = trial_rmse;
                st->best_rmse_known = trial_rmse_known ? 1 : 0;
                st->best_index = (int64_t)i;
                st->best_count = mx;
                on_best(i);
                st->current_iteration = (uint64_t)max_iteration;
            }
        }
    }
    st->count += nvalid;
    st->iterations = end;
}

struct SampleSource {
    Mt19937Mod rng;
    size_t n_points = 0;
    const uint32_t* table = nullptr;
    int m = 3;
    void seed(uint64_t s) { rng.seed((uint32_t)(s & 0xffffffffull)); }
    void fill(size_t begin, size_t end, uint32_t* out) {
        if (table) {
            std::memcpy(out, table + begin * m, sizeof(uint32_t) * (end - begin) * m);
            return;
        }
        if (rng.d != (uint32_t)n_points) rng.set_modulus((uint32_t)n_points);
        const size_t n = end - begin;
        if (m == 3) rng.fill<3>(out, n);
        else if (m == 2) rng.fill<2>(out, n);
        else rng.fill<4>(out, n);
    }
};

static uint32_t pick_splits(uint32_t n_tiles, uint32_t h_pad) {
    const uint32_t groups = h_pad / 64;
    const uint32_t target_wgs = (uint32_t)config().dense_workgroups;
    const uint32_t want = std::max<uint32_t>(1, (target_wgs + n_tiles - 1) / n_tiles);
    return std::min(want, groups);
}

static thread_local int t_dense_fit = 0;
static bool use_dense_scoring() { return t_dense_fit != 0 || config().dense_scoring != 0; }

static uint32_t lead_size() { return (uint32_t)config().lead_hypotheses; }

static size_t chunk_cap_for(const CloudView& v, const SortedView& sv, size_t times = 1) {
    if (!use_dense_scoring()) {
        const size_t by_masks = sv.n_tiles ? std::max<size_t>(((size_t)1 << 30) / ((size_t)sv.n_tiles * 8), 16) * 64 : ~(size_t)0;
        return std::min<size_t>(std::min<size_t>((size_t)config().chunk_cap * times, 262144), by_masks);
    }
    const uint32_t rows = std::max<uint32_t>(1, v.n_pad / kScoreTile);
    const size_t cap = std::min<size_t>(16384, ((size_t)1 << 28) / rows / 64 * 64);
    return std::max<size_t>(cap, 64);
}

static bool bound_pays(uint32_t n_tiles, size_t window_hypotheses) {
    return window_hypotheses >= 8192 && (double)n_tiles * (double)window_hypotheses >= 1.5e7;
}

static bool prestream_enabled() { return config().prestream != 0; }
static int pre_stream_gate(DeviceCtx* ctx) {
    if (!pre_stream_of(ctx) || !ctx->ev_pre_gate) return M3D_OK;
    HIPCHK(hipEventRecord(ctx->ev_pre_gate, ctx->stream));
    HIPCHK(hipStreamWaitEvent(ctx->pre_stream, ctx->ev_pre_gate, 0));
    return M3D_OK;
}

constexpr size_t kBoundTicketWords = 8192;
static int reserve_survivor_scratch(DeviceCtx* ctx, uint32_t h_pad) {
    const size_t words = kBoundTicketWords + (size_t)h_pad + 64;
    if ((size_t)h_pad / 64 + 2 > kBoundTicketWords) return fail(M3D_ERR_INTERNAL, "window too large for the bound's tickets");
    if (ctx->surv_list.cap < sizeof(uint32_t) * words) {
        RESERVE(ctx->surv_list, sizeof(uint32_t) * (kBoundTicketWords + 2 * ((size_t)h_pad + 64)));
        HIPCHK(hipMemsetAsync(ctx->surv_list.p, 0, ctx->surv_list.cap, ctx->stream));
    }
    return M3D_OK;
}
static uint32_t* bound_tickets(DeviceCtx* ctx) { return ctx->surv_list.as<uint32_t>(); }
static uint32_t* bound_list(DeviceCtx* ctx) { return ctx->surv_list.as<uint32_t>() + kBoundTicketWords; }

static int issue_chunk(DeviceCtx* ctx, ChunkSlot& s, const CloudView& v, const SortedView& sv, int kind,
                       double thr, size_t begin, size_t end, SampleSource& src, double* ms_sample,
                       bool prune = false, uint32_t lead = 0, bool new_fit = false ,
                       bool device_records = false ,
                       m3d_comm* comm = nullptr,
                       bool caller_ships_records = false ,
                       const PickFinal* pick_final = nullptr ,
                       bool nothing_to_prune = false ,
                       bool pre = false ,
                       const double* move_best_from = nullptr ) {
    const int m = minimal_sample(kind);
    const uint32_t count = (uint32_t)(end - begin);
    const bool dense = use_dense_scoring();
    pre = pre && !dense && prune && !new_fit && !comm && lead == 0 && !ctx->poison_pending && ctx->pre_stream && s.pre_done;
    hipStream_t st_pre = pre ? ctx->pre_stream : ctx->stream;
    if (move_best_from)
        HIPCHK(hipMemcpyAsync(ctx->best_params.p, move_best_from, sizeof(double) * kModelStride, hipMemcpyDeviceToDevice, st_pre));
    const bool timing = config().kernel_timing != 0;
    if (comm && dense) return fail(M3D_ERR_INVALID_ARG, "sharded fits use the culled scoring path (m3d_config.dense_scoring = 0)");
    const uint32_t world = comm ? (uint32_t)comm->world : 1u, rank = comm ? (uint32_t)comm->rank : 0u;
    const uint32_t sl_pad = round_up((count + world - 1) / world, 64);
    const uint32_t h_pad = comm ? sl_pad * world : round_up(count, 64);
    const uint32_t n_tiles = v.n_pad / kScoreTile;
    if (comm) device_records = true;
    s.begin = begin;
    s.end = end;
    s.h_pad = h_pad;
    RESERVE(s.samples, sizeof(uint32_t) * (size_t)count * m);
    RESERVE(s.score, sizeof(double) * kModelStride * ((size_t)h_pad + 1));
    RESERVE(s.params, sizeof(double) * kModelStride * ((size_t)h_pad + 1));
    RESERVE(s.valid, (size_t)h_pad + 1);
    Cull32Out c32;
    const bool cull32 = !dense && config().cull_fp32 != 0 && sv.radius < 1e18;
    if (cull32) {
        RESERVE(s.cull32, sizeof(float) * 24 * ((size_t)h_pad / 2 + 1));
        c32.out = s.cull32.as<float>();
        for (int k = 0; k < 3; ++k) c32.origin[k] = sv.origin[k];
        c32.radius = sv.radius;
    }
    if (dense || device_records) RESERVE(s.counts, sizeof(uint32_t) * ((size_t)h_pad + 1));
    uint32_t* rec_dev = (!dense && device_records) ? s.counts.as<uint32_t>() : nullptr;
    RESERVE(s.h_samples, sizeof(uint32_t) * (size_t)count * m);
    RESERVE(s.h_counts, sizeof(uint32_t) * ((size_t)h_pad + 4));
    RESERVE(s.h_valid, (size_t)h_pad + 1);
    if (dense) {
        RESERVE(ctx->partial, sizeof(uint32_t) * (size_t)n_tiles * h_pad);
    } else {
        RESERVE(s.masks, sizeof(uint64_t) * (size_t)std::max<uint32_t>(sv.n_tiles, 1) * (h_pad / 64));
        RESERVE(ctx->keep, sizeof(uint64_t) * (size_t)(h_pad / 64));
        RESERVE(ctx->counts_rep, sizeof(uint32_t) * ((size_t)kCountReplicas * h_pad + kPairReplicas));
    }
    const double t0 = now_ms();
    src.fill(begin, end, s.h_samples.as<uint32_t>());
    if (ms_sample) *ms_sample += now_ms() - t0;
    if (!dense && prune) RESERVE(s.ub, sizeof(uint32_t) * 3 * (size_t)h_pad);
    const bool use_lead = !dense && prune && lead >= 64 && lead % 64 == 0 && lead + 64 <= count && (!comm || sl_pad >= lead + 64);
    const bool own_real_ = !comm || (size_t)rank * sl_pad < count;
    LeadPrep lp;
    const bool lead_prepared = use_lead && new_fit && own_real_ && lead <= h_pad && (uint32_t)kPairReplicas <= h_pad;
    const bool all_prepared = nothing_to_prune && !use_lead && lead == 0 && !dense && prune && new_fit && !comm &&
                              (uint32_t)kPairReplicas <= h_pad;
    if (lead_prepared || all_prepared) {
        lp.counts_rep = ctx->counts_rep.as<uint32_t>();
        lp.keep = ctx->keep.as<unsigned long long>();
        lp.rep_stride = h_pad;
        lp.n_rep = kCountReplicas;
        lp.n_lead = all_prepared ? h_pad : lead;
        lp.n_pair = kPairReplicas;
    }
    const bool fit_launched =
        launch_minimal_fit(kind, v, s.h_samples.as<uint32_t>(), count, h_pad + 1, thr, s.score.as<double>(),
                       s.params.as<double>(), s.valid.as<uint8_t>(), st_pre,
                       (!dense && prune) ? s.ub.as<uint32_t>() : nullptr,
                       new_fit ? ctx->best_count.as<uint32_t>() : nullptr, (lead_prepared || all_prepared) ? &lp : nullptr, sv.max_abs,
                       cull32 ? &c32 : nullptr, (ctx->poison_pending && kind == M3D_PLANE) ? &ctx->pending_poison : nullptr,
                       (!dense && prune) ? s.ub.as<uint32_t>() + h_pad : nullptr);
    if (fit_launched && ctx->poison_pending && kind == M3D_PLANE) {
        ctx->poison_pending = false;
        if (ctx->poison_expected_at) *ctx->poison_expected_at += ctx->poison_pending_count;
    }
    if (dense)
        HIPCHK(hipMemsetAsync(s.counts.p, 0, sizeof(uint32_t) * (size_t)h_pad, ctx->stream));
    s.lead_groups = 0;
    s.lead_fused = false;
    s.scored = false;
    s.poll_seq = 0;
    s.host_has_records = true;
    s.done_on_copy_stream = false;
    uint32_t* h_pairs = s.h_counts.as<uint32_t>() + h_pad;
    if (dense) {
        HIPCHK(hipEventRecord(s.k0, ctx->stream));
        launch_score(kind, v, s.score.as<double>(), h_pad, pick_splits(n_tiles, h_pad),
                     ctx->partial.as<uint32_t>(), ctx->stream);
        HIPCHK(hipEventRecord(s.k1, ctx->stream));
        launch_reduce_partials(ctx->partial.as<uint32_t>(), n_tiles, h_pad, s.counts.as<uint32_t>(),
                               ctx->stream);
        s.scored = true;
    } else {
        const uint32_t n_groups = h_pad / 64;
        const uint32_t g0 = comm ? rank * (sl_pad / 64) : 0u, g1 = comm ? g0 + sl_pad / 64 : n_groups;
        const bool own_real = (size_t)g0 * 64 < count;
        uint32_t* ub = prune ? s.ub.as<uint32_t>() : nullptr;
        uint32_t* ubp = (prune && (use_lead || !new_fit) && c32.out && !sv.has_dead && score_phases_for(kind) != 0) ? ub + h_pad : nullptr;
        auto* masks = s.masks.as<unsigned long long>();
        auto* keep = ctx->keep.as<unsigned long long>();
        uint32_t* pair_rep = ctx->counts_rep.as<uint32_t>() + (size_t)kCountReplicas * h_pad;
        uint32_t* bc = prune ? ctx->best_count.as<uint32_t>() : nullptr;
        const bool solo = comm && comm->world == 1 && comm->transport == m3d_comm::kRccl;
        uint32_t* rec_host = (comm && !solo) ? nullptr : s.h_counts.as<uint32_t>();
        PickFinal pfin;
        if (pick_final) {
            pfin = *pick_final;
            pfin.params = s.params.as<double>();
        }
        const uint32_t ga = use_lead ? lead / 64 : 0u;
        if (own_real) {
            s.lead_fused = false;
            if (ga && g0 == 0 && c32.out) {
                if (!lead_prepared)
                    launch_keep_mask(ub, bc, ga, keep, ctx->stream, ctx->counts_rep.as<uint32_t>(), h_pad, 0);
                s.lead_fused = launch_cull_lead(kind, sv, s.score.as<double>(), c32.out, masks, keep, n_groups, ga,
                                                ctx->counts_rep.as<uint32_t>(), h_pad, pair_rep, ub, g1, ctx->stream, ubp);
            }
            const bool bound_on = (kind == M3D_CYLINDER || !ubp) && prune && bc && sv.frames && config().plane_bound != 0 &&
                                  (config().plane_bound == 2 || (kind != M3D_SPHERE && bound_pays(sv.n_tiles, comm ? sl_pad : count))) &&
                                  (use_lead || !new_fit) && std::max(g0, ga) < g1;
            uint32_t* const ubsum = ubp ? ub + 2 * (size_t)h_pad : ub + h_pad;
            if (bound_on) {
                const int src = reserve_survivor_scratch(ctx, h_pad);
                if (src != M3D_OK) return src;
                if (ubp) HIPCHK(hipMemsetAsync(ubsum, 0, sizeof(uint32_t) * h_pad, ctx->stream));
            }
            uint32_t* const surv_count = bound_on ? bc + 6 : nullptr;
            uint32_t* const surv = bound_on ? bound_list(ctx) : nullptr;
            unsigned long long* touched = nullptr;
            bool touched_written = false;
            if (bound_on && kind == M3D_CYLINDER && c32.out && !s.lead_fused && !(ga && g0 >= ga) && g1 - g0 >= 128u) {
                RESERVE(s.touched, sizeof(uint64_t) * (size_t)((sv.n_tiles + 63u) / 64u) * h_pad);
                touched = s.touched.as<unsigned long long>();
            }
            if (!s.lead_fused) {
                if (ga && g0 >= ga)
                    launch_cull_mask(kind, sv, s.score.as<double>(), s.valid.as<uint8_t>(), count, n_groups, masks, ub,
                                     ctx->stream, true, 0, ga, c32.out);
                launch_cull_mask(kind, sv, s.score.as<double>(), s.valid.as<uint8_t>(), count, n_groups, masks, ub, st_pre,
                                 true, g0, g1, c32.out, ubp, touched, h_pad, &touched_written);
            }
            if (pre) {
                HIPCHK(hipEventRecord(s.pre_done, ctx->pre_stream));
                HIPCHK(hipStreamWaitEvent(ctx->stream, s.pre_done, 0));
            }
            uint32_t g_lo = g0;
            if (ga) {
                s.lead_groups = ga;
                g_lo = std::max(g0, ga);
                if (!s.lead_fused) {
                    if (!lead_prepared)
                        launch_keep_mask(ub, bc, ga, keep, ctx->stream, ctx->counts_rep.as<uint32_t>(), h_pad, 0);
                    launch_score_mask(kind, sv, s.score.as<double>(), masks, keep, n_groups, ctx->counts_rep.as<uint32_t>(),
                                      h_pad, pair_rep, ctx->stream, 0, ga, timing ? s.k2 : nullptr, timing ? s.k3 : nullptr);
                }
                launch_lead_fold_keep(ctx->counts_rep.as<uint32_t>(), h_pad, lead, s.valid.as<uint8_t>(), count,
                                      g0 == 0 ? rec_host : nullptr, bc, ub, keep, g1 - g_lo, ctx->stream,
                                      g0 == 0 ? rec_dev : nullptr, g_lo, pick_final ? pick_final->key : nullptr,
                                      pick_final ? pick_final->key2 : nullptr, surv_count, surv);
            } else if (!all_prepared) {
                launch_keep_mask(ub, bc, g1 - g0, keep, ctx->stream, ctx->counts_rep.as<uint32_t>(), h_pad, g0, surv_count, surv);
            }
            if (bound_on)
                launch_plane_bound(kind, sv, s.score.as<double>(), masks, keep, n_groups, g_lo, g1, ubsum, bc, surv_count, surv,
                                   bound_tickets(ctx), c32.out, ctx->stream, config().plane_bound == 2,
                                   touched_written && g_lo == g0 ? touched : nullptr, h_pad);
            bool phased = false;
            if (ubp)
                phased = launch_score_phased(kind, sv, s.score.as<double>(), masks, keep, n_groups, ctx->counts_rep.as<uint32_t>(), h_pad,
                                             pair_rep, ub, ubp, bc, ctx->stream, g_lo, g1, timing ? s.k0 : nullptr, timing ? s.k1 : nullptr);
            if (!phased)
                launch_score_mask(kind, sv, s.score.as<double>(), masks, keep, n_groups, ctx->counts_rep.as<uint32_t>(), h_pad,
                                  pair_rep, ctx->stream, g_lo, g1, timing ? s.k0 : nullptr, timing ? s.k1 : nullptr, bound_on);
            launch_sum_replicas(ctx->counts_rep.as<uint32_t>(), h_pad, g1 * 64u, rec_host, pair_rep, h_pairs,
                                s.valid.as<uint8_t>(), count, bc, ctx->stream, g_lo * 64u, rec_dev, pick_final ? &pfin : nullptr,
                                phased ? keep : nullptr);
            if (pick_final) s.poll_seq = pick_final->seq;
            s.scored = timing;
        } else {
            HIPCHK(hipMemsetAsync(rec_dev + (size_t)g0 * 64, 0, sizeof(uint32_t) * sl_pad, ctx->stream));
            h_pairs[0] = h_pairs[1] = h_pairs[2] = 0;
        }
        if (solo) {
            comm->collectives++;
            s.host_has_records = true;
        } else if (comm) {
            int host_has_all = 0;
            const int rc = comm->allgather_u32_device(rec_dev, sl_pad, ctx->stream, s.h_counts.as<uint32_t>(), &host_has_all);
            if (rc != M3D_OK) return rc;
            s.host_has_records = host_has_all != 0;
            if (!host_has_all && caller_ships_records) {
                HIPCHK(hipEventRecord(ctx->ev_compact, ctx->stream));
                HIPCHK(hipStreamWaitEvent(copy_stream_of(ctx), ctx->ev_compact, 0));
                HIPCHK(hipMemcpyAsync(s.h_counts.p, rec_dev, sizeof(uint32_t) * (size_t)count, hipMemcpyDeviceToHost,
                                      copy_stream_of(ctx)));
                HIPCHK(hipGetLastError());
                HIPCHK(hipEventRecord(s.done, copy_stream_of(ctx)));
                s.host_has_records = true;
                s.done_on_copy_stream = true;
                return M3D_OK;
            }
            if (!host_has_all && !caller_ships_records) {
                HIPCHK(hipMemcpyAsync(s.h_counts.p, rec_dev, sizeof(uint32_t) * (size_t)count, hipMemcpyDeviceToHost,
                                      ctx->stream));
                s.host_has_records = true;
            }
        }
    }
    if (dense)
        HIPCHK(hipMemcpyAsync(s.h_counts.p, s.counts.p, sizeof(uint32_t) * (size_t)count, hipMemcpyDeviceToHost,
                              ctx->stream));
    if (dense) HIPCHK(hipMemcpyAsync(s.h_valid.p, s.valid.p, (size_t)count, hipMemcpyDeviceToHost, ctx->stream));
    HIPCHK(hipGetLastError());
    if (!caller_ships_records && !s.poll_seq) HIPCHK(hipEventRecord(s.done, ctx->stream));
    return M3D_OK;
}

static int wait_pick_seq(DeviceCtx* ctx, uint32_t seq) {
    const volatile uint32_t* p = &ctx->h_pick.as<BestPickHost>()->seq;
    const int spin_us = std::max(config().wait_spin_us, 30);
    const auto t0 = std::chrono::steady_clock::now();
    bool sleeping = false;
    for (uint32_t spins = 1;; ++spins) {
        if ((int32_t)(*p - seq) >= 0) break;
        if (sleeping) {
            std::this_thread::sleep_for(std::chrono::microseconds(20));
            if ((spins & 0x3Fu) == 0) {
                const hipError_t q = hipStreamQuery(ctx->stream);
                if (q == hipSuccess) {
                    if ((int32_t)(*p - seq) >= 0) break;
                    return fail(M3D_ERR_INTERNAL, "the scoring chunk finished without its completion word");
                }
                if (q != hipErrorNotReady) return fail(M3D_ERR_DEVICE, std::string("hipStreamQuery: ") + hipGetErrorString(q));
            }
            continue;
        }
        if ((spins & 0xFFu) == 0 &&
            std::chrono::duration_cast<std::chrono::microseconds>(std::chrono::steady_clock::now() - t0).count() >= spin_us)
            sleeping = true;
#if defined(__x86_64__) || defined(__i386__)
        __builtin_ia32_pause();
#endif
    }
    std::atomic_thread_fence(std::memory_order_acquire);
    return M3D_OK;
}

int stream_wait_spin(DeviceCtx* ctx) {
    const int spin_us = config().wait_spin_us;
// ... 293 lines not shown
                    pending_approx = a_t;
                    return true;
                }
                return false;
            };
            auto on_best = [&](size_t i) {
                best_dev = s.params.as<double>() + (i - s.begin) * kModelStride;
                best_slot = cur;
                best_approx_known = pending_valid;
                best_approx = pending_approx;
                pending_valid = false;
            };
            if (use_dense_scoring())
                replay_range(&out->st, v.n, kind, max_iter, prob, s.begin, s.end, s.h_valid.as<uint8_t>(),
                             s.h_counts.as<uint32_t>(), tie, on_best);
            else if (prob >= 1.0)
                replay_range_exhaustive(&out->st, v.n, kind, max_iter, s.begin, s.end, s.h_counts.as<uint32_t>(), tie, on_best);
            else
                replay_range(&out->st, v.n, kind, max_iter, prob, s.begin, s.end, nullptr, s.h_counts.as<uint32_t>(), tie,
                             on_best);
            if (cb_rc != M3D_OK) {
                rc = cb_rc;
                break;
            }
            if (out->st.stopped) break;
            if (!issued) {
                if (next_begin >= max_iter) break;
                rc = issue_next(cur ^ 1, 0);
                if (rc != M3D_OK) break;
            }
            cur ^= 1;
        }
    }
    if (out->st.best_index < 0) {
        HIPCHK(hipMemsetAsync(ctx->best_params.p, 0, sizeof(double) * kModelStride, ctx->stream));
        best_dev = ctx->best_params.as<double>();
    }
    ctx->last_best_dev = best_dev;
    if (timing_events) out->ms_score = now_ms() - t_score0;
    RESERVE(ctx->h_best, sizeof(double) * 2 * kModelStride);
    if (rc != M3D_OK) {
        (void)hipStreamSynchronize(ctx->stream);
        return rc;
    }
    if (out->internal_error)
        return fail(M3D_ERR_INTERNAL, "scoring kernel and exact evaluation disagree on an inlier count");
    return M3D_OK;
}

int validate_fit_args(int kind, size_t n, bool has_normals, double prob) {
    if (kind == M3D_CYLINDER && !has_normals)
        return fail(M3D_ERR_NO_NORMALS, "Fit cylinder requires normals.");
    if (prob <= 0 || prob > 1 || prob != prob)
        return fail(M3D_ERR_PROBABILITY, "Probability must be > 0 or <= 1.0");
    if (n < (size_t)minimal_sample(kind))
        return fail(M3D_ERR_TOO_FEW_POINTS, "Can not fit model due to lack of points");
    return M3D_OK;
}

uint64_t resolve_seed(const uint64_t* seed) {
    if (seed) return *seed;
    std::random_device rd;
    return rd();
}

int finalize_deferred_refine(DeviceCtx* ctx) {
    DeviceCtx::DeferredRefine& d = ctx->deferred;
    if (!d.pending) return M3D_OK;
    d.pending = false;
    const double* rec = ctx->h_best.as<double>() + (size_t)d.slot * kModelStride;
    uint32_t ni_chk;
    std::memcpy(&ni_chk, ctx->h_pick.as<uint8_t>() + 64 + 8 * d.slot, 4);
    if (ni_chk != d.ni) return fail(M3D_ERR_INTERNAL, "refine pass and scoring kernel disagree on the inlier count");
    double model[4] = {rec[0], rec[1], rec[2], rec[3]};
    const double c0[3] = {rec[4], rec[5], rec[6]};
    double mean[3], sums[14], out[4];
    moments_about_mean(ctx->h_moments.as<double>() + (size_t)d.slot * kFusedMomentDoubles, c0, (double)d.ni, mean, sums + 4);
    if (plane_from_moments(mean, sums + 4, out)) std::memcpy(model, out, sizeof(out));
    std::memcpy(d.params_out, model, sizeof(model));
    return M3D_OK;
}

static int ensure_plane_frames(m3d_cloud* c, int kind, size_t n_hypotheses) {
    const int mode = config().plane_bound;
    if ((kind == M3D_SPHERE && mode != 2) || c->frames_ready || c->frames_failed || mode == 0 || c->work.active || c->n_tiles == 0 ||
        (mode == 1 && (!bound_pays(c->n_tiles, std::min<size_t>(n_hypotheses, chunk_cap_for(c->view(), c->sorted()))) ||
                       (c->one_shot && n_hypotheses < 65536u))))
        return M3D_OK;
    DeviceCtx* ctx = c->ctx;
    HIPCHK(hipSetDevice(ctx->device));
    if (!c->frames.reserve(sizeof(double) * kFrameStride * (size_t)c->n_tiles) ||
        !c->frame_cum.reserve(sizeof(uint16_t) * kCumStride * (size_t)c->n_tiles)) {
        c->frames.release();
        c->frame_cum.release();
        c->frames_failed = true;
        return M3D_OK;
    }
    launch_tile_frames(c->sorted(), c->frames.as<double>(), c->frame_cum.as<uint16_t>(), ctx->stream);
    HIPCHK(hipGetLastError());
    c->frames_ready = true;
    return M3D_OK;
}

int cloud_fit_locked(m3d_cloud* c, int kind, double thr, size_t max_iter, double prob,
                            uint64_t seed, double* params, size_t* inliers, size_t* n_inliers,
                            m3d_stats* stats, const std::function<int(int64_t)>* before_refine_wait,
                            size_t* iterations_hint ,
                            m3d_comm* comm) {
    DeviceCtx* ctx = c->ctx;
    const double t0 = now_ms();
    HIPCHK(hipSetDevice(ctx->device));
    struct DenseGuard {
        int saved;
        explicit DenseGuard(bool on) : saved(t_dense_fit) { if (on) t_dense_fit = 1; }
        ~DenseGuard() { t_dense_fit = saved; }
    } dense_guard(c->n_tiles == 0 && !c->work.active);
    {
        const int frc = ensure_plane_frames(c, kind, max_iter);
        if (frc != M3D_OK) return frc;
    }
    const CloudView v = c->view();
    const CloudView gather = c->base_view();
    const uint32_t* orig = c->orig();
    RansacOut ro;
    uint64_t* idx_host = inliers && !ctx->idx_out_override &&
                                 is_library_pinned(inliers, sizeof(uint64_t) * (size_t)std::max<uint32_t>(v.n, 1))
                             ? reinterpret_cast<uint64_t*>(inliers) : nullptr;
    ctx->compaction_idx_host = nullptr;
    ctx->compaction_fused = false;
    ctx->compaction_mask = false;
    ctx->spec_hit = false;
    ctx->ev_compact_early = false;
    if (ctx->defer_refine) ctx->refine_slot ^= 1;
    int rc = run_ransac(ctx, v, c->sorted(), kind, thr, max_iter, prob, seed, &ro, iterations_hint ? *iterations_hint : 0,
                        orig, comm, idx_host);
    if (rc != M3D_OK) return rc;
    rc = finalize_deferred_refine(ctx);
    if (rc != M3D_OK) return rc;
    if (iterations_hint) *iterations_hint = (size_t)ro.st.iterations;
    const double t1 = now_ms();
    double model[kModelStride] = {0, 0, 0, 0, 0, 0, 0, 0};
    size_t ni = 0;
    int gf_ok = 1;
    const int64_t expected = ro.st.best_index >= 0 ? (int64_t)ro.st.best_count : -1;
    bool refined = false, deferred_now = false;
    if (ctx->spec_compaction) {
        const BestPickHost* ph = ctx->h_pick.as<BestPickHost>();
        const bool hit = !ph->tie && (ro.st.best_index >= 0 ? (ph->have && ph->index == (unsigned long long)ro.st.best_index) : !ph->have);
        ro.spec_hits = hit ? 1 : 0;
        ro.spec_misses = hit ? 0 : 1;
        ctx->spec_hit = hit;
        const bool defer = hit && ctx->defer_refine && !comm && kind == M3D_PLANE && expected >= 3 && ctx->compaction_fused &&
                           inliers && ctx->compaction_idx_host == reinterpret_cast<uint64_t*>(inliers) && before_refine_wait &&
                           (uint64_t)expected <= v.n;
        if (defer) {
            const int hr = (*before_refine_wait)(expected);
            before_refine_wait = nullptr;
            if (hr != M3D_OK) return hr;
            ctx->deferred.pending = true;
            ctx->deferred.slot = refine_slot(ctx);
            ctx->deferred.ni = (uint32_t)expected;
            ctx->deferred.params_out = params;
            ni = (size_t)expected;
            refined = deferred_now = true;
        } else if (hit) {
            rc = refine(ctx, v, gather, orig, kind, thr, ctx->pick.as<BestPick>()->params, model, inliers, &ni, &gf_ok,
                        expected, before_refine_wait, h_best_at(ctx), h_total_at(ctx), true);
// ... 339 lines not shown
    {
        const int frc = ensure_plane_frames(c, kind, end - begin);
        if (frc != M3D_OK) return frc;
    }
    const CloudView v = c->view();
    const SortedView sv = c->sorted();
    const size_t chunk_cap = chunk_cap_for(v, sv);
    SampleSource tsrc;
    tsrc.m = sampler->src.m;
    size_t out = 0;
    struct Pending {
        bool active = false, discard = false;
        size_t out_pos = 0, n = 0;
    } pend[2];
    int cur = 0;
    auto collect = [&](int k) -> int {
        if (!pend[k].active) return M3D_OK;
        ChunkSlot& s = ctx->slot[k];
        HIPCHK(hipEventSynchronize(s.done));
        if (!pend[k].discard) {
            if (valid) {
                unpack_slot(s);
                std::memcpy(counts + pend[k].out_pos, s.h_counts.p, sizeof(uint32_t) * pend[k].n);
                std::memcpy(valid + pend[k].out_pos, s.h_valid.p, pend[k].n);
            } else if (!use_dense_scoring()) {
                std::memcpy(counts + pend[k].out_pos, s.h_counts.p, sizeof(uint32_t) * pend[k].n);
            } else {
                const uint32_t* hc = s.h_counts.as<uint32_t>();
                const uint8_t* hv = s.h_valid.as<uint8_t>();
                for (size_t i = 0; i < pend[k].n; ++i)
                    counts[pend[k].out_pos + i] = hc[i] | (hv[i] ? 0x80000000u : 0u);
            }
        }
        pend[k].active = pend[k].discard = false;
        return M3D_OK;
    };
    size_t j = 0;
    bool first_piece = true;
    const bool prestream_on = prestream_enabled();
    constexpr size_t kFirstPiece = 2048;
    bool first_own = true;
    if (prestream_on && !use_dense_scoring()) {
        const int grc = pre_stream_gate(ctx);
        if (grc != M3D_OK) return grc;
    }
    RESERVE(ctx->best_count, 32);
    RESERVE(ctx->h_inc, 64);
    if (begin == 0) sampler->incumbent = 0;
    *ctx->h_inc.as<uint32_t>() = sampler->incumbent;
    HIPCHK(hipMemcpyAsync(ctx->best_count.p, ctx->h_inc.p, sizeof(uint32_t), hipMemcpyHostToDevice, ctx->stream));
    HIPCHK(hipMemsetAsync(ctx->best_count.as<uint32_t>() + 6, 0, sizeof(uint32_t), ctx->stream));
    {
        const size_t first_own = begin + (size_t)rank * slice;
        if (rank > 0 && first_own < end) {
            const size_t w = std::min<size_t>(std::min<size_t>(lead_size(), chunk_cap), first_own - begin);
            sampler->draw_until(begin + w);
            tsrc.table = sampler->table.data();
            const int rc = issue_chunk(ctx, ctx->slot[cur], v, sv, kind, threshold, begin, begin + w, tsrc, nullptr, true);
            if (rc != M3D_OK) return rc;
            pend[cur].active = pend[cur].discard = true;
            pend[cur].n = w;
            cur ^= 1;
            first_piece = false;
        }
    }
    for (size_t b = begin; b < end; b += slice, ++j) {
        const size_t e = std::min(end, b + slice);
        if (j % world != rank) {
            sampler->draw_until(e);
            continue;
        }
        for (size_t bb = b; bb < e;) {
            const uint32_t lead = first_piece ? lead_size() : 0u;
            first_piece = false;
            const bool short_first = first_own && e - bb > chunk_cap && kFirstPiece >= 2 * (size_t)lead_size();
            const size_t ee = std::min(e, bb + (short_first ? kFirstPiece : chunk_cap));
            const bool pre = prestream_on && !first_own && lead == 0;
            first_own = false;
            sampler->draw_until(ee);
            int rc = collect(cur);
            if (rc != M3D_OK) return rc;
            tsrc.table = sampler->table.data();
            rc = issue_chunk(ctx, ctx->slot[cur], v, sv, kind, threshold, bb, ee, tsrc, nullptr, true, lead, false, false, nullptr, false,
                             nullptr, false, pre);
            if (rc != M3D_OK) return rc;
            pend[cur].active = true;
            pend[cur].out_pos = out;
            pend[cur].n = ee - bb;
            out += ee - bb;
            cur ^= 1;
            bb = ee;
        }
    }
    int rc = collect(0);
    if (rc != M3D_OK) return rc;
    rc = collect(1);
    if (rc != M3D_OK) return rc;
    HIPCHK(hipMemcpyAsync(ctx->h_inc.p, ctx->best_count.p, sizeof(uint32_t), hipMemcpyDeviceToHost, ctx->stream));
    HIPCHK(hipStreamSynchronize(ctx->stream));
    sampler->incumbent = *ctx->h_inc.as<uint32_t>();
    *n_mine = out;
    return M3D_OK;
}

int m3d_bench_time_score(m3d_cloud* c, int kind, double threshold, const uint32_t* samples,
                         size_t n_hypotheses, int reps, int mode, double* ms_avg, uint64_t* listed_pairs) {
    if (!c || kind < 0 || kind > 2 || !samples || !ms_avg || reps < 1 || n_hypotheses == 0 ||
        n_hypotheses > 16384 || mode < 0 || mode > 2)
        return fail(M3D_ERR_INVALID_ARG, "invalid argument");
    if (kind == M3D_CYLINDER && !c->has_normals)
        return fail(M3D_ERR_NO_NORMALS, "Fit cylinder requires normals.");
    DeviceCtx* ctx = c->ctx;
    CtxLock lock(ctx);
    HIPCHK(hipSetDevice(ctx->device));
    const CloudView v = c->view();
    const SortedView sv = c->sorted();
    SampleSource src;
    src.table = samples;
    src.m = minimal_sample(kind);
    ChunkSlot& s = ctx->slot[0];
    int rc = issue_chunk(ctx, s, v, sv, kind, threshold, 0, n_hypotheses, src, nullptr);
    if (rc != M3D_OK) return rc;
    const uint32_t count = (uint32_t)n_hypotheses;
    const uint32_t n_tiles = v.n_pad / kScoreTile;
    RESERVE(ctx->partial, sizeof(uint32_t) * (size_t)n_tiles * s.h_pad);
    const uint32_t n_groups = s.h_pad / 64;
    RESERVE(ctx->masks, sizeof(uint64_t) * (size_t)std::max<uint32_t>(sv.n_tiles, 1) * n_groups);
    RESERVE(ctx->keep, sizeof(uint64_t) * (size_t)n_groups);
    RESERVE(ctx->counts_rep, sizeof(uint32_t) * ((size_t)kCountReplicas * s.h_pad + kPairReplicas));
    RESERVE(ctx->small, 256);
    auto* masks = ctx->masks.as<unsigned long long>();
    auto* keep = ctx->keep.as<unsigned long long>();
    const float* c32 = (!use_dense_scoring() && config().cull_fp32 != 0 && sv.radius < 1e18) ? s.cull32.as<float>() : nullptr;
    launch_cull_mask(kind, sv, s.score.as<double>(), s.valid.as<uint8_t>(), count, n_groups, masks, nullptr, ctx->stream, false, 0,
                     0xFFFFFFFFu, c32);
    launch_keep_mask(nullptr, nullptr, n_groups, keep, ctx->stream);
    if (listed_pairs) {
        launch_count_bits(masks, keep, sv.n_tiles, n_groups, ctx->small.as<unsigned long long>(), ctx->stream);
        unsigned long long tot = 0;
        HIPCHK(hipMemcpyAsync(&tot, ctx->small.p, sizeof(tot), hipMemcpyDeviceToHost, ctx->stream));
        HIPCHK(hipStreamSynchronize(ctx->stream));
        *listed_pairs = tot;
    }
    const uint32_t splits = pick_splits(n_tiles, s.h_pad);
    HIPCHK(hipEventRecord(ctx->ev0, ctx->stream));
    for (int r = 0; r < reps; ++r) {
        if (mode == 0)
            launch_score_mask(kind, sv, s.score.as<double>(), masks, keep, n_groups, ctx->counts_rep.as<uint32_t>(),
                              s.h_pad, ctx->counts_rep.as<uint32_t>() + (size_t)kCountReplicas * s.h_pad, ctx->stream);
        else if (mode == 1)
            launch_cull_mask(kind, sv, s.score.as<double>(), s.valid.as<uint8_t>(), count, n_groups, masks, nullptr,
                             ctx->stream, false, 0, 0xFFFFFFFFu, c32);
        else
            launch_score(kind, v, s.score.as<double>(), s.h_pad, splits, ctx->partial.as<uint32_t>(), ctx->stream);
    }
    HIPCHK(hipEventRecord(ctx->ev1, ctx->stream));
    HIPCHK(hipGetLastError());
    HIPCHK(hipStreamSynchronize(ctx->stream));
    float ms = 0;
    HIPCHK(hipEventElapsedTime(&ms, ctx->ev0, ctx->ev1));
    *ms_avg = (double)ms / reps;
    return M3D_OK;
}

int m3d_bench_upper_bounds(m3d_cloud* c, int kind, double threshold, const uint32_t* samples, size_t n_hypotheses, uint32_t* ub_out);
int m3d_bench_plane_upper_bounds(m3d_cloud* c, double threshold, const uint32_t* samples, size_t n_hypotheses, uint32_t* ub_out) {
    return m3d_bench_upper_bounds(c, M3D_PLANE, threshold, samples, n_hypotheses, ub_out);
}
int m3d_bench_upper_bounds(m3d_cloud* c, int kind, double threshold, const uint32_t* samples, size_t n_hypotheses, uint32_t* ub_out) {
    if (!c || !samples || !ub_out || n_hypotheses == 0 || n_hypotheses > 16384 || kind < M3D_PLANE || kind > M3D_CYLINDER)
        return fail(M3D_ERR_INVALID_ARG, "invalid argument");
    if (kind == M3D_CYLINDER && !c->has_normals) return fail(M3D_ERR_INVALID_ARG, "cylinder hypotheses need normals");
    DeviceCtx* ctx = c->ctx;
    CtxLock lock(ctx);
    HIPCHK(hipSetDevice(ctx->device));
    if (c->work.active || c->n_tiles == 0) return fail(M3D_ERR_INVALID_ARG, "the cloud has no sorted copy of its own");
    if (!c->frames_ready) {
        if (!c->frames.reserve(sizeof(double) * kFrameStride * (size_t)c->n_tiles) ||
            !c->frame_cum.reserve(sizeof(uint16_t) * kCumStride * (size_t)c->n_tiles))
            return fail(M3D_ERR_DEVICE, "out of device memory (tile frames)");
        launch_tile_frames(c->sorted(), c->frames.as<double>(), c->frame_cum.as<uint16_t>(), ctx->stream);
        c->frames_ready = true;
    }
    const CloudView v = c->view();
    const SortedView sv = c->sorted();
    SampleSource src;
    src.table = samples;
    src.m = (uint32_t)minimal_sample(kind);
    ChunkSlot& s = ctx->slot[0];
    int rc = issue_chunk(ctx, s, v, sv, kind, threshold, 0, n_hypotheses, src, nullptr);
    if (rc != M3D_OK) return rc;
    const uint32_t n_groups = s.h_pad / 64;
    RESERVE(ctx->masks, sizeof(uint64_t) * (size_t)std::max<uint32_t>(sv.n_tiles, 1) * n_groups);
    RESERVE(ctx->keep, sizeof(uint64_t) * (size_t)n_groups);
    RESERVE(ctx->small, 256);
    RESERVE(s.ub, sizeof(uint32_t) * 3 * (size_t)s.h_pad);
    rc = reserve_survivor_scratch(ctx, s.h_pad);
    if (rc != M3D_OK) return rc;
    auto* masks = ctx->masks.as<unsigned long long>();
    auto* keep = ctx->keep.as<unsigned long long>();
    uint32_t* ubsum = s.ub.as<uint32_t>() + s.h_pad;
    uint32_t* ctl = ctx->small.as<uint32_t>();
    uint32_t* surv = bound_list(ctx);
    const float* c32 = (!use_dense_scoring() && config().cull_fp32 != 0 && sv.radius < 1e18) ? s.cull32.as<float>() : nullptr;
    HIPCHK(hipMemsetAsync(ubsum, 0, sizeof(uint32_t) * (size_t)s.h_pad, ctx->stream));
    HIPCHK(hipMemsetAsync(ctl, 0, 8, ctx->stream));
    launch_cull_mask(kind, sv, s.score.as<double>(), s.valid.as<uint8_t>(), (uint32_t)n_hypotheses, n_groups, masks, nullptr,
                     ctx->stream, false, 0, 0xFFFFFFFFu, c32);
    launch_keep_mask(nullptr, nullptr, n_groups, keep, ctx->stream, nullptr, 0, 0, ctl + 1, surv);
    launch_plane_bound(kind, sv, s.score.as<double>(), masks, keep, n_groups, 0, n_groups, ubsum, ctl, ctl + 1, surv,
                       bound_tickets(ctx), c32, ctx->stream, true);
    HIPCHK(hipMemcpyAsync(ub_out, ubsum, sizeof(uint32_t) * n_hypotheses, hipMemcpyDeviceToHost, ctx->stream));
    HIPCHK(hipGetLastError());
    HIPCHK(hipStreamSynchronize(ctx->stream));
    return M3D_OK;
}


}
```

Before: 50.20 million.

## Add reference-plane histogram bounds to tighten plane upper bounds

After the lead hypotheses are scored, the best one is taken as a reference plane and each tile gets a histogram of signed distances to it. The histogram is built inside the lead fold/keep kernel as extra blocks. The plane bound kernel then intersects each hypothesis's inlier slab with these histograms, giving a tighter per-tile upper bound (the minimum of the frame bound and the reference bound). Tighter bounds let more hypotheses be culled before exact scoring. The cost is extra histogram work, more shared memory per block in the bound kernel, and a new launch-bounds setting that may affect occupancy.

Result: faster. 58.23 million (median of 6 runs) (+16.0%).

```diff
diff --git a/include/misc3d_amd.h b/include/misc3d_amd.h
--- a/include/misc3d_amd.h
+++ b/include/misc3d_amd.h
@@ -460,6 +460,7 @@
     int32_t lanes_eager;
     int32_t list_mask;
     int32_t mask_early;
+    int32_t ref_bound;
 } m3d_config;
 void m3d_get_config(m3d_config *out);
 int m3d_set_config(const m3d_config *in);
diff --git a/include/misc3d_amd_bench.h b/include/misc3d_amd_bench.h
--- a/include/misc3d_amd_bench.h
+++ b/include/misc3d_amd_bench.h
@@ -18,6 +18,8 @@
 
 int m3d_bench_plane_upper_bounds(m3d_cloud *cloud, double threshold, const uint32_t *samples, size_t n_hypotheses,
                                  uint32_t *ub_out);
+int m3d_bench_plane_ref_upper_bounds(m3d_cloud *cloud, double threshold, const uint32_t *samples, size_t n_hypotheses,
+                                     size_t ref_index, uint32_t *ub_out);
 int m3d_bench_upper_bounds(m3d_cloud *cloud, int kind, double threshold, const uint32_t *samples, size_t n_hypotheses,
                            uint32_t *ub_out);
 int m3d_bench_last_segment_ms(double out[6]);
diff --git a/misc3d_amd/capi.py b/misc3d_amd/capi.py
--- a/misc3d_amd/capi.py
+++ b/misc3d_amd/capi.py
@@ -255,7 +255,7 @@
                                          "reg_neighbour_lists", "reg_prune", "match_brute", "match_fp32_screen",
                                          "pool_limit_mb", "kernel_timing", "reg_sorted_lists", "score_fp32_screen",
                                          "cull_fp32", "reg_fp32_screen", "sorted_tombstones", "score_mfma", "score_mfma_groups", "score_waves4", "score_waves4_groups", "score_phases", "compact_one_pass", "plane_bound",
-                                         "lanes", "wait_spin_us", "prestream", "chunk_cap", "first_chunk", "reg_cells_per_radius", "match_pipeline", "reg_cache", "device_aliases", "lanes_eager", "list_mask", "mask_early")]
+                                         "lanes", "wait_spin_us", "prestream", "chunk_cap", "first_chunk", "reg_cells_per_radius", "match_pipeline", "reg_cache", "device_aliases", "lanes_eager", "list_mask", "mask_early", "ref_bound")]
 
 
 def fp64_issue_rate(device=0, ms_target=2.0):
@@ -641,6 +641,14 @@
         _check(lib().m3d_bench_plane_upper_bounds(self._h, threshold, _p(samples), len(samples), _p(ub)))
         return ub
 
+    def plane_ref_upper_bounds(self, threshold, samples, ref_index):
+        samples = np.ascontiguousarray(samples, dtype=np.uint32).reshape(-1, 3)
+        ub = np.zeros(len(samples), dtype=np.uint32)
+        f = lib().m3d_bench_plane_ref_upper_bounds
+        f.argtypes = [C.c_void_p, C.c_double, C.c_void_p, C.c_size_t, C.c_size_t, C.c_void_p]
+        _check(f(self._h, threshold, _p(samples), len(samples), int(ref_index), _p(ub)))
+        return ub
+
     def upper_bounds(self, kind, threshold, samples):
         samples = np.ascontiguousarray(samples, dtype=np.uint32).reshape(-1, MINIMAL_SAMPLE[kind])
         ub = np.zeros(len(samples), dtype=np.uint32)
diff --git a/misc3d_amd/csrc/m3d_bound.hip b/misc3d_amd/csrc/m3d_bound.hip
--- a/misc3d_amd/csrc/m3d_bound.hip
+++ b/misc3d_amd/csrc/m3d_bound.hip
@@ -204,8 +204,9 @@
 }
 
 constexpr int kBoundWaves = 8;
-template <int KIND , int kBoundTpw >
-__global__ __launch_bounds__(64 * kBoundWaves) void plane_bound_k(const double* __restrict__ frames, const uint16_t* __restrict__ cum,
+template <int KIND , int kBoundTpw ,
+          bool REF >
+__global__ __launch_bounds__(64 * kBoundWaves, REF ? 6 : 1 ) void plane_bound_k(const double* __restrict__ frames, const uint16_t* __restrict__ cum,
                                                                    uint32_t n_tiles, double max_abs,
                                                                    const double* __restrict__ score,
                                                                    const unsigned long long* __restrict__ masks, uint32_t n_groups,
@@ -215,8 +216,12 @@
                                                                    uint32_t* __restrict__ ubsum, const uint32_t* __restrict__ best_count,
                                                                    unsigned long long* __restrict__ keep,
                                                                    uint32_t* __restrict__ tickets ,
-                                                                   uint32_t max_list) {
+                                                                   uint32_t max_list, RefHistArgs ref, bool ref_alone) {
     constexpr int kBoundTpb = kBoundWaves * kBoundTpw;
+    constexpr int kRefTpb = REF ? kBoundTpb : 1;
+    static_assert(!REF || KIND == 0, "reference histograms bound planes");
+    __shared__ double rt_s[kRefTpb][kRefTileStride];
+    __shared__ __attribute__((aligned(8))) uint16_t rcm_s[kRefTpb][kRefCumStride];
     __shared__ float bx_s[kBoundTpb][6];
     __shared__ double c_s[kBoundTpb][3];
     __shared__ float f_s[kBoundTpb][kFrameStride];
@@ -233,6 +238,20 @@
     }
     if (blockIdx.x * 64u >= total) return;
     const uint32_t t0 = blockIdx.y * (uint32_t)kBoundTpb, nt = min((uint32_t)kBoundTpb, n_tiles - t0);
+    double hv[6] = {0.0, 0.0, 0.0, 0.0, 0.0, 0.0};
+    if (REF)
+        for (int k = 0; k < 6; ++k) hv[k] = ref.hdr[k];
+    const bool use_ref = REF && hv[0] != 0.0;
+    RefPlane gp;
+    gp.ok = false;
+    if (REF) {
+        gp = ref_plane_record(hv + 1, max_abs);
+        const double* __restrict__ rsrc = ref.tiles + (size_t)t0 * kRefTileStride;
+        for (uint32_t i = threadIdx.x; i < nt * (uint32_t)kRefTileStride; i += 64u * kBoundWaves) (&rt_s[0][0])[i] = rsrc[i];
+        const uint32_t* __restrict__ csrc = reinterpret_cast<const uint32_t*>(ref.cum + (size_t)t0 * kRefCumStride);
+        uint32_t* cdst = reinterpret_cast<uint32_t*>(&rcm_s[0][0]);
+        for (uint32_t i = threadIdx.x; i < nt * (uint32_t)(kRefCumStride / 2); i += 64u * kBoundWaves) cdst[i] = csrc[i];
+    }
     {
         const double* __restrict__ src = frames + (size_t)t0 * kFrameStride;
         for (uint32_t i = threadIdx.x; i < nt * (uint32_t)kFrameStride; i += 64u * kBoundWaves) {
@@ -272,9 +291,11 @@
         __syncthreads();
         PlaneBoundRec pr;
         CylBoundRec cr;
+        RefHypRec rr;
         if (KIND == 0) {
             pr = plane_bound_record(rec_s[lane], max_abs);
             pr.ok = pr.ok && has;
+            if (REF && use_ref) rr = ref_hyp_record(gp, rec_s[lane], max_abs);
         } else {
             cr = KIND == 1 ? sphere_bound_record(rec_s[lane], max_abs) : cyl_bound_record(rec_s[lane], max_abs);
             cr.ok = cr.ok && has;
@@ -319,8 +340,12 @@
                 tch[i] = has && (uint32_t)tl < nt && live && !(t < 0.0f);
             }
             if (__ballot(tch[i]) == 0ull) continue;
-            const uint32_t u_t = KIND == 0 ? plane_pair_ub(pr, c_s[tl], f_s[tl], cm_s[tl])
-                                           : cyl_pair_ub(cr, c_s[tl], f_s[tl], f_s[tl][0], cm_s[tl]);
+            uint32_t u_t = KIND == 0 ? plane_pair_ub(pr, c_s[tl], f_s[tl], cm_s[tl])
+                                     : cyl_pair_ub(cr, c_s[tl], f_s[tl], f_s[tl][0], cm_s[tl]);
+            if (REF && use_ref) {
+                const uint32_t u_r = ref_pair_ub(rr, pr.a, pr.b, pr.c, pr.d, rt_s[tl], rcm_s[tl]);
+                u_t = ref_alone ? u_r : min(u_t, u_r);
+            }
             ub += tch[i] ? u_t : 0u;
         }
         wsum[wave][lane] = ub;
@@ -440,7 +465,8 @@
 void launch_plane_bound(int kind, const SortedView& s, const double* score, const unsigned long long* masks, unsigned long long* keep,
                         uint32_t n_groups, uint32_t group_begin, uint32_t group_end, uint32_t* ubsum,
                         const uint32_t* best_count, uint32_t* surv_count, const uint32_t* surv, uint32_t* tickets,
-                        const float* cull32, hipStream_t st, bool always, const unsigned long long* touched, uint32_t touched_stride) {
+                        const float* cull32, hipStream_t st, bool always, const unsigned long long* touched, uint32_t touched_stride,
+                        const RefHistArgs* ref, bool ref_alone) {
     group_end = std::min(group_end, n_groups);
     if (!s.frames || !s.frame_cum || !s.n_tiles || !surv || !surv_count || !tickets || group_begin >= group_end) return;
     const uint32_t window = group_end - group_begin;
@@ -459,11 +485,12 @@
     if (s.radius >= 1e18 || kind == 1) cull32 = nullptr;
     auto go = [&](auto kernel) {
         kernel<<<g, b, 0, st>>>(s.frames, s.frame_cum, s.n_tiles, s.max_abs, score, masks, n_groups, s.boxes, cull32, surv_count, surv,
-                                ubsum, best_count, keep, tickets, max_list);
+                                ubsum, best_count, keep, tickets, max_list, (ref && kind == 0) ? *ref : RefHistArgs{}, ref_alone);
     };
-    if (kind == 0) go(plane_bound_k<0, tpw>);
-    else if (kind == 1) go(plane_bound_k<1, tpw_cyl>);
-    else go(plane_bound_k<2, tpw_cyl>);
-}
-
-}
+    if (kind == 0 && ref) go(plane_bound_k<0, tpw, true>);
+    else if (kind == 0) go(plane_bound_k<0, tpw, false>);
+    else if (kind == 1) go(plane_bound_k<1, tpw_cyl, false>);
+    else go(plane_bound_k<2, tpw_cyl, false>);
+}
+
+}
diff --git a/misc3d_amd/csrc/m3d_bound_fp.hpp b/misc3d_amd/csrc/m3d_bound_fp.hpp
--- a/misc3d_amd/csrc/m3d_bound_fp.hpp
+++ b/misc3d_amd/csrc/m3d_bound_fp.hpp
@@ -201,4 +201,81 @@
     return framed ? u_t : (uint32_t)kBoundTilePoints;
 }
 
-}
+#ifndef M3D_REF_BINS
+#define M3D_REF_BINS 64
+#endif
+constexpr int kRefBins = M3D_REF_BINS;
+constexpr int kRefCumStride = kRefBins + 4;
+constexpr int kRefTileStride = 5;
+constexpr int kRefHdrDoubles = 8;
+constexpr double kRefMinCos = 0.9;
+static_assert(kRefBins >= 8 && kRefBins <= 128 && kRefBins % 8 == 0, "8 .. 128 bins");
+
+struct RefPlane {
+    double a, b, c, d, invw, n2, n1, Mg;
+    bool ok;
+};
+M3D_HD RefPlane ref_plane_record(const double* rec , double max_abs) {
+    RefPlane g;
+    g.a = rec[0]; g.b = rec[1]; g.c = rec[2]; g.d = rec[3];
+    const double T = rec[4];
+    g.n1 = (fabs(g.a) + fabs(g.b)) + fabs(g.c);
+    g.n2 = (g.a * g.a + g.b * g.b) + g.c * g.c;
+    g.Mg = g.n1 * max_abs + fabs(g.d);
+    g.invw = (double)(kRefBins / 8) / T;
+    g.ok = (T > 1e-12) && (T < 1e12) && (g.n1 > 1e-12) && (g.n1 < 1e12) && (g.Mg < 1e12);
+    return g;
+}
+M3D_HD int ref_bin_of(double t ) {
+    return (int)fmin(fmax(floor(t), (double)(-kRefBins / 2 - 1)), (double)(kRefBins / 2)) + (kRefBins / 2 + 1);
+}
+M3D_HD int ref_bin(double s, double invw) { return ref_bin_of(s * invw); }
+struct RefHypRec {
+    double alpha, sa , w0, np;
+    bool flip, ok;
+};
+M3D_HD RefHypRec ref_hyp_record(const RefPlane& g, const double* rec , double max_abs) {
+    RefHypRec r;
+    const double dot = (rec[0] * g.a + rec[1] * g.b) + rec[2] * g.c;
+    r.flip = dot < 0.0;
+    const double sg = r.flip ? -1.0 : 1.0;
+    const double a = sg * rec[0], b = sg * rec[1], c = sg * rec[2], d = sg * rec[3], T = rec[4];
+    r.alpha = fabs(dot) / g.n2;
+    r.sa = (1.0 / r.alpha) * g.invw;
+    const double n1 = (fabs(a) + fabs(b)) + fabs(c), n2 = (a * a + b * b) + c * c;
+    const double Mh = n1 * max_abs + fabs(d);
+    const double qa = a - r.alpha * g.a, qb = b - r.alpha * g.b, qc = c - r.alpha * g.c;
+#ifdef M3D_BOUND_NO_SLACK
+    r.np = sqrt((qa * qa + qb * qb) + qc * qc);
+    r.w0 = T;
+#else
+    r.np = (sqrt((qa * qa + qb * qb) + qc * qc) * (1.0 + 1e-12) + 1e-15 * (r.alpha * g.n1 + n1)) * (1.0 + 1e-11);
+    r.w0 = (T * (1.0 + 1e-12) + 1e-13 * (Mh + r.alpha * g.Mg)) * (1.0 + 1e-11);
+#endif
+    r.ok = g.ok && (T > 1e-12) && (T < 1e12) && (n1 > 1e-12) && (n1 < 1e12) && (Mh < 1e12) &&
+           (dot * dot >= (kRefMinCos * kRefMinCos) * (n2 * g.n2)) && (r.alpha > 1e-12) && (r.alpha < 1e12);
+    return r;
+}
+template <class CumPtr>
+M3D_HD uint32_t ref_pair_ub(const RefHypRec& r, double a, double b, double c, double d, const double* t, CumPtr cm) {
+    const double sc = ((a * t[0] + b * t[1]) + c * t[2]) + d;
+    const double K = (r.flip ? -sc : sc) - r.alpha * t[3];
+    const double w = r.w0 + r.np * t[4];
+    double tl = (-K - w) * r.sa, th = (-K + w) * r.sa;
+#ifndef M3D_BOUND_NO_SLACK
+    tl -= 1e-11 * fabs(tl);
+    th += 1e-11 * fabs(th);
+#endif
+    const bool whole = !(tl == tl) || !(th == th);
+    const int bl = ref_bin_of(whole ? 0.0 : tl), bh = ref_bin_of(whole ? 0.0 : th);
+#ifdef M3D_BOUND_NO_SLACK
+    const int lo_c = (int)cm[bl + 1], hi_c = (int)cm[bh];
+#else
+    const int lo_c = (int)cm[bl], hi_c = (int)cm[bh + 1];
+#endif
+    uint32_t u_t = (uint32_t)(hi_c > lo_c ? hi_c - lo_c : 0);
+    u_t = whole ? (uint32_t)cm[kRefBins + 2] : u_t;
+    return r.ok ? u_t : (uint32_t)kBoundTilePoints;
+}
+
+}
diff --git a/misc3d_amd/csrc/m3d_config.cpp b/misc3d_amd/csrc/m3d_config.cpp
--- a/misc3d_amd/csrc/m3d_config.cpp
+++ b/misc3d_amd/csrc/m3d_config.cpp
@@ -50,6 +50,7 @@
     if (c.list_mask < 0) c.list_mask = 1;
     if (c.list_mask > 16) c.list_mask = 16;
     c.mask_early = c.mask_early != 0;
+    if (c.ref_bound < 0 || c.ref_bound > 2) c.ref_bound = 1;
 }
 void load_env() {
     std::memset(&g_cfg, 0, sizeof(g_cfg));
@@ -84,6 +85,7 @@
     g_cfg.lanes_eager = (int32_t)env_long("M3D_LANES_EAGER", 2);
     g_cfg.list_mask = (int32_t)env_long("M3D_LIST_MASK", 1);
     g_cfg.mask_early = !env_is("M3D_MASK_EARLY", '0');
+    g_cfg.ref_bound = (int32_t)env_long("M3D_REF_BOUND", 1);
     sanitize(g_cfg);
 }
 }
diff --git a/misc3d_amd/csrc/m3d_cull_kernels.hip b/misc3d_amd/csrc/m3d_cull_kernels.hip
--- a/misc3d_amd/csrc/m3d_cull_kernels.hip
+++ b/misc3d_amd/csrc/m3d_cull_kernels.hip
@@ -8,6 +8,7 @@
 
 #include "m3d_config.hpp"
 #include "m3d_fp.hpp"
+#include "m3d_ref_hist.hpp"
 #include "m3d_tile_count.hpp"
 #include "m3d_wave.hpp"
 
@@ -512,7 +513,12 @@
                                                         uint32_t* __restrict__ records_dev,
                                                         unsigned long long* __restrict__ pick_key,
                                                         unsigned long long* __restrict__ pick_key2,
-                                                        SurvOut surv) {
+                                                        SurvOut surv, uint32_t n_keep_groups, RefHistArgs ref) {
+    __shared__ uint32_t hist[kRefHistWords];
+    if (blockIdx.x >= n_keep_groups) {
+        ref_hist_tile(ref, blockIdx.x - n_keep_groups, hist);
+        return;
+    }
     const uint32_t g = group_offset + blockIdx.x;
     const uint32_t prev = best_count[0];
     uint32_t v = 0;
@@ -561,11 +567,20 @@
 void launch_lead_fold_keep(const uint32_t* counts_rep, uint32_t rep_stride, uint32_t lead, const uint8_t* valid,
                            uint32_t h_count, uint32_t* records, uint32_t* best_count, const uint32_t* ub,
                            unsigned long long* keep, uint32_t n_groups_rest, hipStream_t st, uint32_t* records_dev,
-                           uint32_t group_begin, unsigned long long* pick_key, unsigned long long* pick_key2, uint32_t* surv_count, uint32_t* surv) {
+                           uint32_t group_begin, unsigned long long* pick_key, unsigned long long* pick_key2, uint32_t* surv_count, uint32_t* surv,
+                           const RefHistArgs* ref) {
     if (group_begin == 0xFFFFFFFFu) group_begin = lead / 64u;
     if (!n_groups_rest) return;
-    lead_fold_keep_k<<<n_groups_rest, 64, 0, st>>>(counts_rep, rep_stride, lead, valid, h_count, records, best_count, ub,
-                                                   keep, const_cast<uint32_t*>(counts_rep), group_begin, records_dev, pick_key, pick_key2, SurvOut{surv_count, surv});
+    lead_fold_keep_k<<<n_groups_rest + (ref ? ref->n_tiles : 0u), 64, 0, st>>>(counts_rep, rep_stride, lead, valid, h_count, records, best_count, ub,
+                                                   keep, const_cast<uint32_t*>(counts_rep), group_begin, records_dev, pick_key, pick_key2, SurvOut{surv_count, surv},
+                                                   n_groups_rest, ref ? *ref : RefHistArgs{});
+}
+__global__ __launch_bounds__(64) void ref_hist_k(RefHistArgs ref) {
+    __shared__ uint32_t hist[kRefHistWords];
+    ref_hist_tile(ref, blockIdx.x, hist);
+}
+void launch_ref_hist(const RefHistArgs& a, hipStream_t st) {
+    if (a.n_tiles) ref_hist_k<<<a.n_tiles, 64, 0, st>>>(a);
 }
 
 template <int KIND>
diff --git a/misc3d_amd/csrc/m3d_cull_kernels.hpp b/misc3d_amd/csrc/m3d_cull_kernels.hpp
--- a/misc3d_amd/csrc/m3d_cull_kernels.hpp
+++ b/misc3d_amd/csrc/m3d_cull_kernels.hpp
@@ -26,13 +26,40 @@
 
 constexpr int kTileF32Floats = 3 * kTilePoints;
 void launch_tile_frames(const SortedView& s, double* frames, uint16_t* cum, hipStream_t st);
+struct RefHistArgs {
+    const double* sx = nullptr;
+    const double* sy = nullptr;
+    const double* sz = nullptr;
+    uint32_t n_tiles = 0;
+    const double* score = nullptr;
+    const uint32_t* counts_rep = nullptr;
+    uint32_t rep_stride = 0, lead = 0;
+    const uint8_t* valid = nullptr;
+    uint32_t h_count = 0, fixed_index = 0;
+    uint32_t min_count = 1;
+    double max_abs = 0.0;
+    double* hdr = nullptr;
+    double* tiles = nullptr;
+    uint16_t* cum = nullptr;
+};
+inline size_t ref_hist_bytes(uint32_t n_tiles) {
+    return sizeof(double) * (kRefHdrDoubles + (size_t)kRefTileStride * n_tiles) + sizeof(uint16_t) * (size_t)kRefCumStride * n_tiles;
+}
+inline void ref_hist_place(RefHistArgs& a, void* block) {
+    a.hdr = static_cast<double*>(block);
+    a.tiles = a.hdr + kRefHdrDoubles;
+    a.cum = reinterpret_cast<uint16_t*>(a.tiles + (size_t)kRefTileStride * a.n_tiles);
+}
+void launch_ref_hist(const RefHistArgs& a, hipStream_t st);
 void launch_plane_bound(int kind, const SortedView& s, const double* score, const unsigned long long* masks, unsigned long long* keep,
                         uint32_t n_groups, uint32_t group_begin, uint32_t group_end, uint32_t* ubsum,
                         const uint32_t* best_count, uint32_t* surv_count, const uint32_t* surv, uint32_t* tickets,
                         const float* cull32, hipStream_t st,
                         bool always = false ,
                         const unsigned long long* touched = nullptr ,
-                        uint32_t touched_stride = 0);
+                        uint32_t touched_stride = 0,
+                        const RefHistArgs* ref = nullptr ,
+                        bool ref_alone = false );
 void launch_tile_boxes(const SortedView& s, double* boxes, hipStream_t st);
 PoisonJob make_poison_job(const SortedView& s, const double* model, double thr, uint32_t* total);
 void launch_poison_plane_inliers(const PoisonJob& job, hipStream_t st);
@@ -107,7 +134,8 @@
                            uint32_t group_begin = 0xFFFFFFFFu ,
                            unsigned long long* pick_key = nullptr ,
                            unsigned long long* pick_key2 = nullptr ,
-                           uint32_t* surv_count = nullptr, uint32_t* surv = nullptr );
+                           uint32_t* surv_count = nullptr, uint32_t* surv = nullptr ,
+                           const RefHistArgs* ref = nullptr );
 void launch_count_bits(const unsigned long long* masks, const unsigned long long* keep, uint32_t n_tiles,
                        uint32_t n_groups, unsigned long long* total, hipStream_t st);
 
diff --git a/misc3d_amd/csrc/m3d_driver.hpp b/misc3d_amd/csrc/m3d_driver.hpp
--- a/misc3d_amd/csrc/m3d_driver.hpp
+++ b/misc3d_amd/csrc/m3d_driver.hpp
@@ -148,6 +148,7 @@
     PinBuf h_reg;
     uint32_t sync_seq = 0;
     DevBuf surv_list;
+    DevBuf ref_hist;
     hipEvent_t ev0 = nullptr, ev1 = nullptr;
     PinBuf h_match;
     std::vector<hipEvent_t> aux_events;
diff --git a/misc3d_amd/csrc/m3d_fit.cpp b/misc3d_amd/csrc/m3d_fit.cpp
--- a/misc3d_amd/csrc/m3d_fit.cpp
+++ b/misc3d_amd/csrc/m3d_fit.cpp
@@ -146,6 +146,10 @@
 static bool bound_pays(uint32_t n_tiles, size_t window_hypotheses) {
     return window_hypotheses >= 8192 && (double)n_tiles * (double)window_hypotheses >= 1.5e7;
 }
+static int bound_mode(int kind) {
+    const int mode = config().plane_bound;
+    return (mode != 0 && kind == M3D_PLANE && config().ref_bound == 2) ? 2 : mode;
+}
 
 static bool prestream_enabled() { return config().prestream != 0; }
 static int pre_stream_gate(DeviceCtx* ctx) {
@@ -177,7 +181,8 @@
                        const PickFinal* pick_final = nullptr ,
                        bool nothing_to_prune = false ,
                        bool pre = false ,
-                       const double* move_best_from = nullptr ) {
+                       const double* move_best_from = nullptr ,
+                       bool first_of_stream = false ) {
     const int m = minimal_sample(kind);
     const uint32_t count = (uint32_t)(end - begin);
     const bool dense = use_dense_scoring();
@@ -291,9 +296,26 @@
                 s.lead_fused = launch_cull_lead(kind, sv, s.score.as<double>(), c32.out, masks, keep, n_groups, ga,
                                                 ctx->counts_rep.as<uint32_t>(), h_pad, pair_rep, ub, g1, ctx->stream, ubp);
             }
-            const bool bound_on = (kind == M3D_CYLINDER || !ubp) && prune && bc && sv.frames && config().plane_bound != 0 &&
-                                  (config().plane_bound == 2 || (kind != M3D_SPHERE && bound_pays(sv.n_tiles, comm ? sl_pad : count))) &&
+            const bool bound_on = (kind == M3D_CYLINDER || !ubp) && prune && bc && sv.frames && bound_mode(kind) != 0 &&
+                                  (bound_mode(kind) == 2 || (kind != M3D_SPHERE && bound_pays(sv.n_tiles, comm ? sl_pad : count))) &&
                                   (use_lead || !new_fit) && std::max(g0, ga) < g1;
+            const bool ref_on = bound_on && kind == M3D_PLANE && !ubp && !comm && (new_fit || first_of_stream) && use_lead && ga && g0 == 0 && !sv.has_dead &&
+                                config().ref_bound != 0 && (config().ref_bound == 2 || bound_pays(sv.n_tiles, count));
+            RefHistArgs ref;
+            if (ref_on) {
+                RESERVE(ctx->ref_hist, ref_hist_bytes(sv.n_tiles));
+                ref.sx = sv.x; ref.sy = sv.y; ref.sz = sv.z;
+                ref.n_tiles = sv.n_tiles;
+                ref.score = s.score.as<double>();
+                ref.counts_rep = ctx->counts_rep.as<uint32_t>();
+                ref.rep_stride = h_pad;
+                ref.lead = lead;
+                ref.valid = s.valid.as<uint8_t>();
+                ref.h_count = count;
+                ref.max_abs = sv.max_abs;
+                ref.min_count = config().ref_bound == 2 ? 1u : 8u * sv.n_tiles;
+                ref_hist_place(ref, ctx->ref_hist.p);
+            }
             uint32_t* const ubsum = ubp ? ub + 2 * (size_t)h_pad : ub + h_pad;
             if (bound_on) {
                 const int src = reserve_survivor_scratch(ctx, h_pad);
@@ -332,14 +354,14 @@
                 launch_lead_fold_keep(ctx->counts_rep.as<uint32_t>(), h_pad, lead, s.valid.as<uint8_t>(), count,
                                       g0 == 0 ? rec_host : nullptr, bc, ub, keep, g1 - g_lo, ctx->stream,
                                       g0 == 0 ? rec_dev : nullptr, g_lo, pick_final ? pick_final->key : nullptr,
-                                      pick_final ? pick_final->key2 : nullptr, surv_count, surv);
+                                      pick_final ? pick_final->key2 : nullptr, surv_count, surv, ref_on ? &ref : nullptr);
             } else if (!all_prepared) {
                 launch_keep_mask(ub, bc, g1 - g0, keep, ctx->stream, ctx->counts_rep.as<uint32_t>(), h_pad, g0, surv_count, surv);
             }
             if (bound_on)
                 launch_plane_bound(kind, sv, s.score.as<double>(), masks, keep, n_groups, g_lo, g1, ubsum, bc, surv_count, surv,
-                                   bound_tickets(ctx), c32.out, ctx->stream, config().plane_bound == 2,
-                                   touched_written && g_lo == g0 ? touched : nullptr, h_pad);
+                                   bound_tickets(ctx), c32.out, ctx->stream, bound_mode(kind) == 2,
+                                   touched_written && g_lo == g0 ? touched : nullptr, h_pad, ref_on ? &ref : nullptr);
             bool phased = false;
             if (ubp)
                 phased = launch_score_phased(kind, sv, s.score.as<double>(), masks, keep, n_groups, ctx->counts_rep.as<uint32_t>(), h_pad,
@@ -799,7 +821,7 @@
 }
 
 static int ensure_plane_frames(m3d_cloud* c, int kind, size_t n_hypotheses) {
-    const int mode = config().plane_bound;
+    const int mode = bound_mode(kind);
     if ((kind == M3D_SPHERE && mode != 2) || c->frames_ready || c->frames_failed || mode == 0 || c->work.active || c->n_tiles == 0 ||
         (mode == 1 && (!bound_pays(c->n_tiles, std::min<size_t>(n_hypotheses, chunk_cap_for(c->view(), c->sorted()))) ||
                        (c->one_shot && n_hypotheses < 65536u))))
@@ -1305,7 +1327,7 @@
             if (rc != M3D_OK) return rc;
             tsrc.table = sampler->table.data();
             rc = issue_chunk(ctx, ctx->slot[cur], v, sv, kind, threshold, bb, ee, tsrc, nullptr, true, lead, false, false, nullptr, false,
-                             nullptr, false, pre);
+                             nullptr, false, pre, nullptr, world == 1 && bb == 0);
             if (rc != M3D_OK) return rc;
             pend[cur].active = true;
             pend[cur].out_pos = out;
@@ -1390,7 +1412,18 @@
 int m3d_bench_plane_upper_bounds(m3d_cloud* c, double threshold, const uint32_t* samples, size_t n_hypotheses, uint32_t* ub_out) {
     return m3d_bench_upper_bounds(c, M3D_PLANE, threshold, samples, n_hypotheses, ub_out);
 }
+static int bench_upper_bounds(m3d_cloud* c, int kind, double threshold, const uint32_t* samples, size_t n_hypotheses, uint32_t* ub_out,
+                              long ref_index);
 int m3d_bench_upper_bounds(m3d_cloud* c, int kind, double threshold, const uint32_t* samples, size_t n_hypotheses, uint32_t* ub_out) {
+    return bench_upper_bounds(c, kind, threshold, samples, n_hypotheses, ub_out, -1);
+}
+int m3d_bench_plane_ref_upper_bounds(m3d_cloud* c, double threshold, const uint32_t* samples, size_t n_hypotheses, size_t ref_index,
+                                     uint32_t* ub_out) {
+    if (ref_index >= n_hypotheses) return fail(M3D_ERR_INVALID_ARG, "invalid argument");
+    return bench_upper_bounds(c, M3D_PLANE, threshold, samples, n_hypotheses, ub_out, (long)ref_index);
+}
+static int bench_upper_bounds(m3d_cloud* c, int kind, double threshold, const uint32_t* samples, size_t n_hypotheses, uint32_t* ub_out,
+                              long ref_index) {
     if (!c || !samples || !ub_out || n_hypotheses == 0 || n_hypotheses > 16384 || kind < M3D_PLANE || kind > M3D_CYLINDER)
         return fail(M3D_ERR_INVALID_ARG, "invalid argument");
     if (kind == M3D_CYLINDER && !c->has_normals) return fail(M3D_ERR_INVALID_ARG, "cylinder hypotheses need normals");
@@ -1431,8 +1464,19 @@
     launch_cull_mask(kind, sv, s.score.as<double>(), s.valid.as<uint8_t>(), (uint32_t)n_hypotheses, n_groups, masks, nullptr,
                      ctx->stream, false, 0, 0xFFFFFFFFu, c32);
     launch_keep_mask(nullptr, nullptr, n_groups, keep, ctx->stream, nullptr, 0, 0, ctl + 1, surv);
+    RefHistArgs ref;
+    if (ref_index >= 0) {
+        RESERVE(ctx->ref_hist, ref_hist_bytes(sv.n_tiles));
+        ref.sx = sv.x; ref.sy = sv.y; ref.sz = sv.z;
+        ref.n_tiles = sv.n_tiles;
+        ref.score = s.score.as<double>();
+        ref.fixed_index = (uint32_t)ref_index;
+        ref.max_abs = sv.max_abs;
+        ref_hist_place(ref, ctx->ref_hist.p);
+        launch_ref_hist(ref, ctx->stream);
+    }
     launch_plane_bound(kind, sv, s.score.as<double>(), masks, keep, n_groups, 0, n_groups, ubsum, ctl, ctl + 1, surv,
-                       bound_tickets(ctx), c32, ctx->stream, true);
+                       bound_tickets(ctx), c32, ctx->stream, true, nullptr, 0, ref_index >= 0 ? &ref : nullptr, true);
     HIPCHK(hipMemcpyAsync(ub_out, ubsum, sizeof(uint32_t) * n_hypotheses, hipMemcpyDeviceToHost, ctx->stream));
     HIPCHK(hipGetLastError());
     HIPCHK(hipStreamSynchronize(ctx->stream));
diff --git a/misc3d_amd/csrc/m3d_ref_hist.hpp b/misc3d_amd/csrc/m3d_ref_hist.hpp
--- /dev/null
+++ b/misc3d_amd/csrc/m3d_ref_hist.hpp
@@ -0,0 +1,101 @@
+#pragma once
+#include "m3d_bound_fp.hpp"
+#include "m3d_cull_kernels.hpp"
+#include "m3d_wave.hpp"
+
+namespace m3d {
+
+constexpr int kRefHistPerLane = (kRefBins + 3 + 63) / 64;
+constexpr int kRefHistWords = 64 * kRefHistPerLane;
+
+__device__ __forceinline__ void ref_hist_tile(const RefHistArgs& a, uint32_t tile, uint32_t* hist ) {
+    const int lane = threadIdx.x & 63;
+    uint32_t hg = a.fixed_index;
+    bool have = true;
+    if (a.counts_rep) {
+        unsigned long long key = 0;
+        for (uint32_t h = lane; h < a.lead; h += 64u) {
+            uint32_t c = 0;
+#pragma unroll
+            for (int r = 0; r < kCountReplicas; ++r) c += a.counts_rep[(size_t)r * a.rep_stride + h];
+            const bool ok = h < a.h_count && a.valid[h];
+            if (ok && c) key = max(key, ((unsigned long long)c << 32) | (0xFFFFFFFFu - h));
+        }
+        key = wave_max(key);
+        have = key != 0ull && (uint32_t)(key >> 32) >= a.min_count;
+        hg = 0xFFFFFFFFu - (uint32_t)key;
+    }
+    hg = (uint32_t)__builtin_amdgcn_readfirstlane((int)hg);
+    RefPlane g;
+    g.ok = false;
+    if (have) g = ref_plane_record(a.score + (size_t)hg * kModelStride, a.max_abs);
+    have = have && g.ok;
+    if (tile == 0 && lane == 0) {
+        a.hdr[0] = have ? 1.0 : 0.0;
+        if (have)
+            for (int k = 0; k < 5; ++k) a.hdr[1 + k] = a.score[(size_t)hg * kModelStride + k];
+        a.hdr[6] = (double)hg;
+    }
+    if (!have) return;
+    constexpr int P = kTilePoints / 64;
+    double px[P], py[P], pz[P];
+    bool fin[P];
+    double lo[3] = {INFINITY, INFINITY, INFINITY}, hi[3] = {-INFINITY, -INFINITY, -INFINITY};
+    uint32_t nf = 0;
+#pragma unroll
+    for (int j = 0; j < P; ++j) {
+        const size_t i = (size_t)tile * kTilePoints + j * 64 + lane;
+        px[j] = a.sx[i];
+        py[j] = a.sy[i];
+        pz[j] = a.sz[i];
+        fin[j] = (px[j] * 0.0 == 0.0) && (py[j] * 0.0 == 0.0) && (pz[j] * 0.0 == 0.0);
+        if (fin[j]) {
+            lo[0] = fmin(lo[0], px[j]); hi[0] = fmax(hi[0], px[j]);
+            lo[1] = fmin(lo[1], py[j]); hi[1] = fmax(hi[1], py[j]);
+            lo[2] = fmin(lo[2], pz[j]); hi[2] = fmax(hi[2], pz[j]);
+            ++nf;
+        }
+    }
+    for (int k = 0; k < 3; ++k) {
+        lo[k] = wave_min(lo[k]);
+        hi[k] = wave_max(hi[k]);
+    }
+    nf = wave_sum(nf);
+    double c[3] = {0.0, 0.0, 0.0};
+    if (nf)
+        for (int k = 0; k < 3; ++k) c[k] = 0.5 * lo[k] + 0.5 * hi[k];
+    for (int i = lane; i < kRefHistWords; i += 64) hist[i] = 0u;
+    __syncthreads();
+    double r2 = 0.0;
+#pragma unroll
+    for (int j = 0; j < P; ++j) {
+        if (!fin[j]) continue;
+        const double dx = px[j] - c[0], dy = py[j] - c[1], dz = pz[j] - c[2];
+        r2 = fmax(r2, (dx * dx + dy * dy) + dz * dz);
+        const double s = ((g.a * px[j] + g.b * py[j]) + g.c * pz[j]) + g.d;
+        atomicAdd(&hist[ref_bin(s, g.invw)], 1u);
+    }
+    r2 = wave_max(r2);
+    __syncthreads();
+    {
+        uint32_t own = 0;
+#pragma unroll
+        for (int i = 0; i < kRefHistPerLane; ++i) own += hist[lane * kRefHistPerLane + i];
+        uint32_t run = wave_incl_scan(own, lane) - own;
+        uint16_t* __restrict__ cm = a.cum + (size_t)tile * kRefCumStride;
+#pragma unroll
+        for (int i = 0; i < kRefHistPerLane; ++i) {
+            const int idx = lane * kRefHistPerLane + i;
+            if (idx <= kRefBins + 2) cm[idx] = (uint16_t)run;
+            run += hist[idx];
+        }
+    }
+    if (lane == 0) {
+        double* __restrict__ t = a.tiles + (size_t)tile * kRefTileStride;
+        t[0] = c[0]; t[1] = c[1]; t[2] = c[2];
+        t[3] = ((g.a * c[0] + g.b * c[1]) + g.c * c[2]) + g.d;
+        t[4] = sqrt(r2) * (1.0 + 1e-12);
+    }
+}
+
+}
```
